# dash-robotics/perception

Hardware: AMD Instinct MI355X
Metric: frames/sec (640x480 D435 cloud, plane+cluster+ICP) (higher is better)
Workload: dtype f32

## Files before the change

perception_amd/csrc/common.hpp:

```cpp
#pragma once
#include <hip/hip_runtime.h>
#include <stdint.h>

#include "../../include/cuboid_hip.h"

namespace cd {

constexpr int WAVE = 64;
constexpr int BLOCK = 256;
constexpr int WAVES_PER_BLOCK = BLOCK / WAVE;
constexpr int ITEMS = 8;
constexpr int TILE = BLOCK * ITEMS;
constexpr int WAVE_SPAN = WAVE * ITEMS;
constexpr int RADIX_BITS = 8;
constexpr int RADIX = 1 << RADIX_BITS;
#ifndef CD_SORT_BLOCK
#define CD_SORT_BLOCK 1024
#endif
constexpr int SORT_BLOCK = CD_SORT_BLOCK;
constexpr int SORT_TILE = SORT_BLOCK * ITEMS;
#ifndef CD_SCATTER_BLOCK
#define CD_SCATTER_BLOCK 512
#endif
constexpr int SCATTER_BLOCK = CD_SCATTER_BLOCK;
constexpr int SCATTER_TILE = SCATTER_BLOCK * ITEMS;
constexpr int RUN_SHIFT = 20;
constexpr uint32_t RUN_START_MASK = (1u << RUN_SHIFT) - 1u;
constexpr int KICP = CD_MAX_CLUSTERS_PER_FRAME;
constexpr int FIX_SHIFT = 32;
constexpr int FIX_SHIFT_D2 = 36;
constexpr int RND_TABLE = 1 << 15;
constexpr int SAMPLER_MAP = 8192;
constexpr int MAX_HYP = 1024 + 16;
constexpr int CELL_BUCKETS = 1 << 16;
constexpr int ICP_TPL_CHUNK = 2048;
constexpr int ICP_SUB = 64;
#ifndef CD_PIPE_SLOTS
#define CD_PIPE_SLOTS 4
#endif
static_assert(CD_PIPE_SLOTS >= 1 && CD_PIPE_SLOTS <= 6, "LDS budget of k_icp_pipe");
constexpr int ICP_TPL_LDS = CD_PIPE_SLOTS <= 2 ? 7616 : 7552;
constexpr int ICP_MAX_CELLS = 12288;
constexpr int ICP_CELL_STRIDE = ICP_MAX_CELLS + 8;
constexpr int ICP_MAX_CHUNKS = 12;
constexpr int ICP_BIG_MAX = 65535;
constexpr int ICP_BIG_PATCHES = 1024;
constexpr int ICP_QSLICE = 512;

struct FrameState {
    int32_t status;
    int32_t n_c;
    uint32_t mn[3], mx[3];
    int32_t min_b[3], div_b[3];
    int32_t key_bits;
    int32_t n_v;
    int32_t n_plane;
    int32_t n_o;
    int32_t n_k;
    int32_t n_hyp;
    int32_t sampler_exhausted;
    int32_t ksize[KICP];
    int32_t koff[KICP];
    float origin[3];
    int32_t n_cropped;
    int32_t cl_done;
    int32_t crop_overflow;
    int32_t scan_stalled;
    int32_t n_runs;
    int32_t digit_vary;
    int32_t pad_;
};

struct CropLimits {
    float zlo, zhi, xlo, xhi;
};

struct KeyPack {
    int32_t enabled;
    int32_t bi, bj;
    int32_t ilo, jlo, klo;
};

struct BBoxGate {
    double P[12];
    float rect[4];
    int32_t enable;
    int32_t pad;
};

struct IcpCluster {
    int32_t src_off;
    int32_t n;
    int32_t frame, k;
    int32_t tpl_off, tpl_m;
    int32_t tile0;
    int32_t slot;
};

struct IcpGrid {
    float ox, oy, oz, inv;
    float cell;
    int32_t nx, ny, nz;
    int32_t ncell;
    int32_t cell_off;
    int32_t kd_split;
    int32_t pad;
    float half_lo[2][4], half_hi[2][4];
    int32_t nchunk;
    int32_t chunk_start[ICP_MAX_CHUNKS], chunk_n[ICP_MAX_CHUNKS];
    int32_t pad2[3];
    float chunk_lo[ICP_MAX_CHUNKS][4], chunk_hi[ICP_MAX_CHUNKS][4];
};

struct IcpSuper {
    int32_t n;
    int32_t first[64], cnt[64];
    float lo[64][4], hi[64][4];
};

constexpr int LAT_MAX_FACES = 6;
constexpr int LAT_MAX_TAB = 512;
struct IcpLattice {
    int32_t nface;
    int32_t ntab;
    int32_t n[3];
    int32_t toff[3];
    float noi[3], inv[3];
    int32_t w[LAT_MAX_FACES];
    int32_t fast[LAT_MAX_FACES];
    int32_t base[LAT_MAX_FACES];
    float c[LAT_MAX_FACES];
    uint32_t m0[LAT_MAX_FACES], m1[LAT_MAX_FACES], m2[LAT_MAX_FACES];
    int32_t axis_face[3];
    float axis_c[3];
    int32_t axes_distinct;
    float4 tab[LAT_MAX_TAB];
};

inline void lattice_classify_axes(IcpLattice* L) {
    uint32_t nan_bits = 0x7fc00000u;
    float nan;
    static_assert(sizeof(nan) == sizeof(nan_bits), "float32");
    __builtin_memcpy(&nan, &nan_bits, sizeof(nan));
    for (int a = 0; a < 3; ++a) { L->axis_face[a] = -1; L->axis_c[a] = nan; }
    L->axes_distinct = 0;
    if (L->nface < 1 || L->nface > 3) return;
    for (int f = 0; f < L->nface; ++f) {
        const int w = L->w[f];
        if (w < 0 || w > 2 || L->axis_face[w] >= 0) {
            for (int a = 0; a < 3; ++a) { L->axis_face[a] = -1; L->axis_c[a] = nan; }
            return;
        }
        L->axis_face[w] = f; L->axis_c[w] = L->c[f];
    }
    L->axes_distinct = 1;
}

struct IcpState {
    float Tfinal[16];
    float T[16];
    double prev_mse;
    int32_t iters;
    int32_t done;
    int32_t converged;
    int32_t status;
};

struct IcpWork {
    int32_t cluster, tile;
};

struct IcpParams {
    int32_t max_iter;
    float grid_rc;
    double trans_eps, rel_mse, rot_thr, abs_mse;
    int32_t pipe_slots;
    int32_t donate;
    int32_t* don;
    int32_t don_idle;
    int32_t don_fault;
};
struct IcpBound {
    float d2_max;
    int32_t bounded;
    uint32_t* ncorr;
};
constexpr int DON_AVAIL = 0;
constexpr int DON_FINISHED = 1;
constexpr int DON_TAIL = 2;
constexpr int DON_HEAD = 3;
constexpr int DON_ERR = 4;
constexpr int DON_BOX = 16;
constexpr int DON_CAP = 2048;

#ifdef __HIPCC__
#ifndef CD_NO_FRONT_PRIO
#define CD_FRONT_PRIO() __builtin_amdgcn_s_setprio(3)
#else
#define CD_FRONT_PRIO()
#endif
__device__ __forceinline__ uint32_t f2ord(float f) {
    const uint32_t u = __float_as_uint(f);
    return (u & 0x80000000u) ? ~u : (u | 0x80000000u);
}
__host__ __device__ __forceinline__ float ord2f(uint32_t o) {
    const uint32_t u = (o & 0x80000000u) ? (o & 0x7fffffffu) : ~o;
#ifdef __HIP_DEVICE_COMPILE__
    return __uint_as_float(u);
#else
    float f;
    __builtin_memcpy(&f, &u, 4);
    return f;
#endif
}
__device__ __forceinline__ uint64_t ballot64(bool p) { return __builtin_amdgcn_ballot_w64(p); }
#ifdef CD_BOUNDS
__device__ __forceinline__ bool cd_in_range(bool ok, unsigned code) {
    if (!ok) printf("cuboid_hip BOUNDS: check %u failed in workgroup %u thread %u\n", code, (unsigned)blockIdx.x, (unsigned)threadIdx.x);
    return ok;
}
#define CD_IN_RANGE(cond, code) cd::cd_in_range((cond), (code))
#else
#define CD_IN_RANGE(cond, code) true
#endif
template <int R, typename T>
__device__ __forceinline__ void load_rows_clamped(const T* __restrict__ a, int first, int n, T (&v)[R]) {
#pragma unroll
    for (int j = 0; j < R; ++j) {
        int e = first + j * WAVE;
        e = e < n ? e : n - 1;
        v[j] = a[e < 0 ? 0 : e];
    }
}

__device__ __forceinline__ uint64_t lanemask_lt() {
    const uint32_t lane = threadIdx.x & 63;
    return (lane == 0) ? 0ull : (~0ull >> (64 - lane));
}
template <int R>
__device__ __forceinline__ int tile_prefix(const uint64_t (&bal)[R], int (&s_cnt)[WAVES_PER_BLOCK], int* total) {
    const int w = threadIdx.x >> 6, lane = threadIdx.x & 63;
    int wtot = 0;
#pragma unroll
    for (int j = 0; j < R; ++j) wtot += __popcll(bal[j]);
    __syncthreads();
    if (lane == 0) s_cnt[w] = wtot;
    __syncthreads();
    int pos = 0, tot = 0;
    for (int q = 0; q < WAVES_PER_BLOCK; ++q) { if (q < w) pos += s_cnt[q]; tot += s_cnt[q]; }
    *total = tot;
    return pos;
}
__device__ __forceinline__ long long fixq(float v, int shift) {
    return __double2ll_rn(ldexp((double)v, shift));
}
__device__ __forceinline__ unsigned long long fixq_fast(float v, int shift) {
    const double u = __dadd_rn(ldexp((double)v, shift), 6755399441055744.0);
    const unsigned long long b = (unsigned long long)__double_as_longlong(u);
    const int hi = __builtin_amdgcn_sbfe((int)(unsigned)(b >> 32), 0, 19);
    return ((unsigned long long)(unsigned)hi << 32) | (unsigned)b;
}
#define CD_DPP_ADD2(a, b, ctrl)                                                                                   \
    asm volatile("s_nop 1\n\t"                                                                                    \
                 "v_add_co_u32_dpp %0, vcc, %0, %0 " ctrl " row_mask:0xf bank_mask:0xf bound_ctrl:0\n\t"         \
                 "v_addc_co_u32_dpp %1, vcc, %1, %1, vcc " ctrl " row_mask:0xf bank_mask:0xf bound_ctrl:0\n\t"   \
                 "v_add_co_u32_dpp %2, vcc, %2, %2 " ctrl " row_mask:0xf bank_mask:0xf bound_ctrl:0\n\t"         \
                 "v_addc_co_u32_dpp %3, vcc, %3, %3, vcc " ctrl " row_mask:0xf bank_mask:0xf bound_ctrl:0"        \
                 : "+v"(a##lo), "+v"(a##hi), "+v"(b##lo), "+v"(b##hi)::"vcc")
__device__ __forceinline__ void wave_fold_to_lds(const unsigned long long (&S)[16], int nsum, unsigned long long* dst) {
    const int lane = threadIdx.x & 63;
#pragma unroll
    for (int k = 0; k < 16; k += 2) {
        if (k < nsum) {
            unsigned xlo = (unsigned)S[k], xhi = (unsigned)(S[k] >> 32), ylo = (unsigned)S[k + 1], yhi = (unsigned)(S[k + 1] >> 32);
            CD_DPP_ADD2(x, y, "row_shr:1");
            CD_DPP_ADD2(x, y, "row_shr:2");
            CD_DPP_ADD2(x, y, "row_shr:4");
            CD_DPP_ADD2(x, y, "row_shr:8");
            if ((lane & 15) == 15) {
                atomicAdd(&dst[k], ((unsigned long long)xhi << 32) | xlo);
                if (k + 1 < nsum) atomicAdd(&dst[k + 1], ((unsigned long long)yhi << 32) | ylo);
            }
        }
    }
}

__device__ __forceinline__ unsigned long long wave_sum_u64(unsigned long long v) {
#pragma unroll
    for (int o = 32; o > 0; o >>= 1) v += __shfl_xor(v, o, 64);
    return v;
}
__device__ __forceinline__ int wave_sum_i32(int v) {
#pragma unroll
    for (int o = 32; o > 0; o >>= 1) v += __shfl_xor(v, o, 64);
    return v;
}
__device__ __forceinline__ float dist2(float ax, float ay, float az, float bx, float by, float bz) {
    const float dx = ax - bx, dy = ay - by, dz = az - bz;
    return __fadd_rn(__fadd_rn(__fmul_rn(dx, dx), __fmul_rn(dy, dy)), __fmul_rn(dz, dz));
}
constexpr int TICKET_PITCH = 32;
__device__ __forceinline__ int take_ticket(int* counter, int tickets, int* s_ticket) {
    if (threadIdx.x == 0) {
        const int t = __hip_atomic_fetch_add(counter, 1, __ATOMIC_RELAXED, __HIP_MEMORY_SCOPE_AGENT);
        if (t == tickets - 1) __hip_atomic_store(counter, 0, __ATOMIC_RELAXED, __HIP_MEMORY_SCOPE_AGENT);
        *s_ticket = CD_IN_RANGE(t >= 0 && t < tickets, 1u) ? t : 0;
    }
    __syncthreads();
    return *s_ticket;
}
__device__ __forceinline__ int chained_scan(int* state, int stride, int tile, int tot, int* gave_up) {
    unsigned* st = reinterpret_cast<unsigned*>(state);
    const unsigned FLAG_TOTAL = 1u << 30, FLAG_PREFIX = 2u << 30, VALUE = (1u << 30) - 1u;
    int excl = 0;
    if (tile > 0) {
        __hip_atomic_store(st + (size_t)tile * stride, FLAG_TOTAL | (unsigned)tot, __ATOMIC_RELAXED, __HIP_MEMORY_SCOPE_AGENT);
        for (int q = tile - 1; q >= 0; --q) {
            unsigned v;
            int spins = 0;
            do {
                v = __hip_atomic_load(st + (size_t)q * stride, __ATOMIC_RELAXED, __HIP_MEMORY_SCOPE_AGENT);
                if (++spins > (1 << 20)) { *gave_up = 1; v = FLAG_PREFIX; }
            } while ((v & (FLAG_TOTAL | FLAG_PREFIX)) == 0u);
            excl += (int)(v & VALUE);
            if (v & FLAG_PREFIX) break;
        }
    }
    __hip_atomic_store(st + (size_t)tile * stride, FLAG_PREFIX | (unsigned)(excl + tot), __ATOMIC_RELAXED, __HIP_MEMORY_SCOPE_AGENT);
    return excl;
}
__device__ __forceinline__ void chained_scan2(unsigned long long* state, int tile, int tot_a, int tot_b, int* excl_a, int* excl_b,
                                              int* gave_up) {
    const unsigned long long FLAG_TOTAL = 1ull << 62, FLAG_PREFIX = 2ull << 62, MASK = (1ull << 31) - 1ull;
    unsigned long long ea = 0ull, eb = 0ull;
    if (tile > 0) {
        __hip_atomic_store(state + tile, FLAG_TOTAL | ((unsigned long long)(unsigned)tot_b << 31) | (unsigned long long)(unsigned)tot_a,
                           __ATOMIC_RELAXED, __HIP_MEMORY_SCOPE_AGENT);
        for (int q = tile - 1; q >= 0; --q) {
            unsigned long long v;
            int spins = 0;
            do {
                v = __hip_atomic_load(state + q, __ATOMIC_RELAXED, __HIP_MEMORY_SCOPE_AGENT);
                if (++spins > (1 << 20)) { *gave_up = 1; v = FLAG_PREFIX; }
            } while ((v & (FLAG_TOTAL | FLAG_PREFIX)) == 0ull);
            ea += v & MASK;
            eb += (v >> 31) & MASK;
            if (v & FLAG_PREFIX) break;
        }
    }
    __hip_atomic_store(state + tile, FLAG_PREFIX | ((eb + (unsigned long long)(unsigned)tot_b) << 31) | (ea + (unsigned long long)(unsigned)tot_a),
                       __ATOMIC_RELAXED, __HIP_MEMORY_SCOPE_AGENT);
    *excl_a = (int)ea;
    *excl_b = (int)eb;
}
__device__ __forceinline__ float plane_dist(float a, float b, float c, float d, float x, float y, float z) {
    return fabsf(__fadd_rn(__fadd_rn(__fmul_rn(a, x), __fmul_rn(b, y)), __fadd_rn(__fmul_rn(c, z), d)));
}
#endif

}
```

perception_amd/csrc/k_plane.hip:

```cpp
#include <algorithm>

#include "extract_flags.hpp"
#include "kernels.hpp"

namespace cd {

constexpr int SAMPLER_MAP_SMALL = 1024;
constexpr int SAMPLER_SMALL_HYP = 64;
static_assert(3 * (SAMPLER_SMALL_HYP - 1) + 3 + 6 <= (SAMPLER_MAP_SMALL * 3) / 4,
              "the small map holds the slots of SAMPLER_SMALL_HYP hypotheses without a rejected sample: 3 + 3 (h - 1) before the last draw, which asks for 6 more");
static_assert(2 * SAMPLER_MAP_SMALL * sizeof(int) <= 8 * 1024 && 2 * SAMPLER_MAP <= CELL_BUCKETS, "8 KiB of LDS; the spill area is the frame's part of the cluster hash heads");

struct SamplerState {
    int rp, h, used, it, exhausted;
};

template <int MAP>
__device__ __forceinline__ bool sampler_run(int* key, int* val, SamplerState& st, const float4* __restrict__ P, int n,
                                            const int* __restrict__ rnd, int h_target, float4* __restrict__ M, int* __restrict__ V) {
    auto slot = [&](int pos) {
        uint32_t h = ((uint32_t)pos * 2654435761u) & (MAP - 1);
        while (key[h] != -1 && key[h] != pos) h = (h + 1) & (MAP - 1);
        return (int)h;
    };
    int rp = st.rp, h = st.h, used = st.used, it0 = st.it, exhausted = 0;
    auto get = [&](int pos) { const int h = slot(pos); return key[h] == pos ? val[h] : pos; };
    auto set = [&](int pos, int v) { const int h = slot(pos); if (key[h] == -1) ++used; key[h] = pos; val[h] = v; };
    while (h < h_target) {
        bool good = false;
        int s0 = 0, s1 = 0, s2 = 0;
        for (int it = it0; it < 1000; ++it) {
            if (rp + 3 > RND_TABLE || used + 6 > (SAMPLER_MAP * 3) / 4) { exhausted = 1; break; }
            if (MAP < SAMPLER_MAP && used + 6 > (MAP * 3) / 4) { st.rp = rp; st.h = h; st.used = used; st.it = it; return false; }
            for (int i = 0; i < 3; ++i) {
                const uint32_t r = (uint32_t)rnd[rp++];
                const int j = i + (int)(r % (uint32_t)(n - i));
                const int vi = get(i), vj = get(j);
                set(i, vj); set(j, vi);
            }
            s0 = get(0); s1 = get(1); s2 = get(2);
            const float4 p0 = P[s0], p1 = P[s1], p2 = P[s2];
            const float q0 = __fdiv_rn(p1.x - p0.x, p2.x - p0.x);
            const float q1 = __fdiv_rn(p1.y - p0.y, p2.y - p0.y);
            const float q2 = __fdiv_rn(p1.z - p0.z, p2.z - p0.z);
            if ((q0 != q1) || (q2 != q1)) { good = true; break; }
        }
        it0 = 0;
        if (!good) { exhausted = 1; break; }
        const float4 p0 = P[s0], p1 = P[s1], p2 = P[s2];
        const float ax = p1.x - p0.x, ay = p1.y - p0.y, az = p1.z - p0.z;
        const float bx = p2.x - p0.x, by = p2.y - p0.y, bz = p2.z - p0.z;
        const float q0 = __fdiv_rn(ax, bx), q1 = __fdiv_rn(ay, by), q2 = __fdiv_rn(az, bz);
        int ok = 1;
        float4 m = make_float4(0.f, 0.f, 0.f, 0.f);
        if (q0 == q1 && q2 == q1) {
            ok = 0;
        } else {
            float mx = __fsub_rn(__fmul_rn(ay, bz), __fmul_rn(az, by));
            float my = __fsub_rn(__fmul_rn(az, bx), __fmul_rn(ax, bz));
            float mz = __fsub_rn(__fmul_rn(ax, by), __fmul_rn(ay, bx));
            const float nrm = __fsqrt_rn(__fadd_rn(__fadd_rn(__fmul_rn(mx, mx), __fmul_rn(my, my)), __fmul_rn(mz, mz)));
            mx = __fdiv_rn(mx, nrm); my = __fdiv_rn(my, nrm); mz = __fdiv_rn(mz, nrm);
            const float d = __fmul_rn(-1.0f, __fadd_rn(__fadd_rn(__fmul_rn(mx, p0.x), __fmul_rn(my, p0.y)), __fmul_rn(mz, p0.z)));
            m = make_float4(mx, my, mz, d);
        }
        M[h] = m;
        V[h] = ok;
        ++h;
    }
    st.rp = rp; st.h = h; st.used = used; st.it = 0; st.exhausted = exhausted;
    return true;
}

template <int MAP>
__global__ void __launch_bounds__(WAVE) k_ransac_sample(const float4* __restrict__ vox, int N,
                                                        FrameState* __restrict__ fs, const int* __restrict__ rnd,
                                                        int h_target, const int* __restrict__ active,
                                                        float4* __restrict__ models, int* __restrict__ valid,
                                                        int* __restrict__ spill, int spill_pitch) {
    CD_FRONT_PRIO();
    __shared__ int s_key[MAP];
    __shared__ int s_val[MAP];
    const int f = blockIdx.x;
    if (active && !active[f]) return;
    for (int i = threadIdx.x; i < MAP; i += WAVE) s_key[i] = -1;
    __syncthreads();
    if (threadIdx.x != 0) return;
    const int n = fs[f].n_v;
    const float4* P = vox + (size_t)f * N;
    float4* M = models + (size_t)f * MAX_HYP;
    int* V = valid + (size_t)f * MAX_HYP;
    if (n < 3) { fs[f].n_hyp = 0; fs[f].sampler_exhausted = 1; return; }
    SamplerState st = {0, 0, 0, 0, 0};
    const bool finished = sampler_run<MAP>(s_key, s_val, st, P, n, rnd, h_target, M, V);
    if (MAP < SAMPLER_MAP && !finished) {
        int* g_key = spill + (size_t)f * spill_pitch;
        int* g_val = g_key + SAMPLER_MAP;
        for (int i = 0; i < SAMPLER_MAP; ++i) g_key[i] = -1;
        for (int i = 0; i < MAP; ++i) {
            const int pos = s_key[i];
            if (pos == -1) continue;
            uint32_t h = ((uint32_t)pos * 2654435761u) & (SAMPLER_MAP - 1);
            while (g_key[h] != -1) h = (h + 1) & (SAMPLER_MAP - 1);
            g_key[h] = pos;
            g_val[h] = s_val[i];
        }
        sampler_run<SAMPLER_MAP>(g_key, g_val, st, P, n, rnd, h_target, M, V);
    }
    fs[f].n_hyp = st.h;
    fs[f].sampler_exhausted = st.exhausted;
}

__global__ void __launch_bounds__(BLOCK) k_ransac_count(const float4* __restrict__ vox, int N,
                                                        const FrameState* __restrict__ fs,
                                                        const float4* __restrict__ models, const int* __restrict__ valid,
                                                        const int* __restrict__ active, int h0, int h1, float thr,
                                                        int* __restrict__ counts) {
    CD_FRONT_PRIO();
    const int f = blockIdx.y, tile = blockIdx.x, w = threadIdx.x >> 6, lane = threadIdx.x & 63;
    if (active && !active[f]) return;
    const int n = fs[f].n_v;
    if (tile * TILE >= n) return;
    const int hmax = min(h1, fs[f].n_hyp);
    const float4* P = vox + (size_t)f * N;
    const int base = tile * TILE + w * WAVE_SPAN + lane;
    float px[ITEMS], py[ITEMS], pz[ITEMS];
    bool in[ITEMS];
#pragma unroll
    for (int j = 0; j < ITEMS; ++j) {
        const int e = base + j * WAVE;
        in[j] = e < n;
        const float4 p = P[e < n ? e : n - 1];
        px[j] = p.x; py[j] = p.y; pz[j] = p.z;
    }
    const float4* M = models + (size_t)f * MAX_HYP;
    const int* V = valid + (size_t)f * MAX_HYP;
    for (int h = h0; h < hmax; ++h) {
        if (!V[h]) continue;
        const float4 m = M[h];
        int c = 0;
#pragma unroll
        for (int j = 0; j < ITEMS; ++j)
            c += __popcll(__ballot(in[j] && plane_dist(m.x, m.y, m.z, m.w, px[j], py[j], pz[j]) < thr));
        if (lane == 0 && c) atomicAdd(&counts[(size_t)f * MAX_HYP + h], c);
    }
}

__global__ void __launch_bounds__(BLOCK) k_plane_cov(const float4* __restrict__ vox, int N,
                                                     const FrameState* __restrict__ fs, const float4* __restrict__ model,
                                                     const int* __restrict__ have, float thr,
                                                     unsigned long long* __restrict__ sums) {
    CD_FRONT_PRIO();
    const int f = blockIdx.y, tile = blockIdx.x, w = threadIdx.x >> 6, lane = threadIdx.x & 63;
    const int n = fs[f].n_v;
    if (tile * TILE >= n || !have[f]) return;
    const float4 m = model[f];
    const float4* P = vox + (size_t)f * N;
    const int base = tile * TILE + w * WAVE_SPAN + lane;
    unsigned long long S[10] = {0, 0, 0, 0, 0, 0, 0, 0, 0, 0};
    float4 pr[ITEMS];
    load_rows_clamped<ITEMS>(P, base, n, pr);
#pragma unroll
    for (int j = 0; j < ITEMS; ++j) {
        const int e = base + j * WAVE;
        if (e < n) {
            const float4 p = pr[j];
            if (plane_inlier(m, 1, thr, p)) {
                S[0] += (unsigned long long)fixq(__fmul_rn(p.x, p.x), FIX_SHIFT);
                S[1] += (unsigned long long)fixq(__fmul_rn(p.x, p.y), FIX_SHIFT);
                S[2] += (unsigned long long)fixq(__fmul_rn(p.x, p.z), FIX_SHIFT);
                S[3] += (unsigned long long)fixq(__fmul_rn(p.y, p.y), FIX_SHIFT);
                S[4] += (unsigned long long)fixq(__fmul_rn(p.y, p.z), FIX_SHIFT);
                S[5] += (unsigned long long)fixq(__fmul_rn(p.z, p.z), FIX_SHIFT);
                S[6] += (unsigned long long)fixq(p.x, FIX_SHIFT);
                S[7] += (unsigned long long)fixq(p.y, FIX_SHIFT);
                S[8] += (unsigned long long)fixq(p.z, FIX_SHIFT);
                S[9] += 1ull;
            }
        }
    }
#pragma unroll
    for (int k = 0; k < 10; ++k) {
        const unsigned long long t = wave_sum_u64(S[k]);
        if (lane == 0 && t) atomicAdd(&sums[(size_t)f * 10 + k], t);
    }
}

__global__ void __launch_bounds__(BLOCK) k_plane_flag_count(const float4* __restrict__ vox, int N, int T,
                                                            const FrameState* __restrict__ fs,
                                                            const float4* __restrict__ model, const int* __restrict__ have,
                                                            float thr, int negative, int crop2, float z2lo, float z2hi, BBoxGate gate,
                                                            FrameRects rects, int* __restrict__ cnt_plane, int* __restrict__ cnt_obj) {
    CD_FRONT_PRIO();
    __shared__ int s_a[WAVES_PER_BLOCK], s_b[WAVES_PER_BLOCK];
    const int f = blockIdx.y, tile = blockIdx.x, w = threadIdx.x >> 6, lane = threadIdx.x & 63;
    const int n = fs[f].n_v;
    if (tile * TILE >= n) return;
    frame_rect(gate, rects, f);
    const float4 m = model[f];
    const int hv = have[f];
    const float4* P = vox + (size_t)f * N;
    const int base = tile * TILE + w * WAVE_SPAN + lane;
    int ca = 0, cb = 0;
    float4 pr[ITEMS];
    load_rows_clamped<ITEMS>(P, base, n, pr);
#pragma unroll
    for (int j = 0; j < ITEMS; ++j) {
        const int e = base + j * WAVE;
        bool inl = false, obj = false;
        if (e < n) extract_flags(m, hv, thr, negative, crop2, z2lo, z2hi, gate, pr[j], inl, obj);
        ca += __popcll(__ballot(inl));
        cb += __popcll(__ballot(obj));
    }
    if (lane == 0) { s_a[w] = ca; s_b[w] = cb; }
    __syncthreads();
    if (threadIdx.x == 0) {
        cnt_plane[(size_t)f * T + tile] = s_a[0] + s_a[1] + s_a[2] + s_a[3];
        cnt_obj[(size_t)f * T + tile] = s_b[0] + s_b[1] + s_b[2] + s_b[3];
    }
}

__global__ void __launch_bounds__(BLOCK) k_extract_scatter(const float4* __restrict__ vox, int N, int T,
                                                           const FrameState* __restrict__ fs,
                                                           const float4* __restrict__ model, const int* __restrict__ have,
                                                           float thr, int negative, int crop2, float z2lo, float z2hi, BBoxGate gate,
                                                           FrameRects rects, const int* __restrict__ off_plane, const int* __restrict__ off_obj,
                                                           int* __restrict__ plane_idx, float4* __restrict__ obj_out) {
    CD_FRONT_PRIO();
    __shared__ int s_a[WAVES_PER_BLOCK], s_b[WAVES_PER_BLOCK];
    const int f = blockIdx.y, tile = blockIdx.x, w = threadIdx.x >> 6, lane = threadIdx.x & 63;
    const int n = fs[f].n_v;
    if (tile * TILE >= n) return;
    frame_rect(gate, rects, f);
    const size_t fbase = (size_t)f * N;
    const float4 m = model[f];
    const int hv = have[f];
    const float4* P = vox + fbase;
    const int base = tile * TILE + w * WAVE_SPAN + lane;
    float4 p[ITEMS];
    uint64_t ba[ITEMS], bb[ITEMS];
    int ca = 0, cb = 0;
    load_rows_clamped<ITEMS>(P, base, n, p);
#pragma unroll
    for (int j = 0; j < ITEMS; ++j) {
        const int e = base + j * WAVE;
        bool inl = false, obj = false;
        if (e < n) extract_flags(m, hv, thr, negative, crop2, z2lo, z2hi, gate, p[j], inl, obj);
        ba[j] = __ballot(inl);
        bb[j] = __ballot(obj);
        ca += __popcll(ba[j]);
        cb += __popcll(bb[j]);
    }
    if (lane == 0) { s_a[w] = ca; s_b[w] = cb; }
    __syncthreads();
    int pa = off_plane[(size_t)f * T + tile], pb = off_obj[(size_t)f * T + tile];
    for (int q = 0; q < w; ++q) { pa += s_a[q]; pb += s_b[q]; }
    const uint64_t lt = lanemask_lt();
#pragma unroll
    for (int j = 0; j < ITEMS; ++j) {
        const int e = base + j * WAVE;
        if ((ba[j] >> lane) & 1ull) plane_idx[fbase + pa + __popcll(ba[j] & lt)] = e;
        if ((bb[j] >> lane) & 1ull) obj_out[fbase + pb + __popcll(bb[j] & lt)] = p[j];
        pa += __popcll(ba[j]);
        pb += __popcll(bb[j]);
    }
}

void launch_ransac_sample(hipStream_t s, const float4* vox, int N, int F, FrameState* fs, const int* rnd_table,
                          int h_target, const int* active, float4* models, int* valid, int* spill, int spill_pitch) {
    if (spill && spill_pitch >= 2 * SAMPLER_MAP && h_target <= SAMPLER_SMALL_HYP)
        hipLaunchKernelGGL(k_ransac_sample<SAMPLER_MAP_SMALL>, dim3(F), dim3(WAVE), 0, s, vox, N, fs, rnd_table, h_target, active, models, valid, spill, spill_pitch);
    else
        hipLaunchKernelGGL(k_ransac_sample<SAMPLER_MAP>, dim3(F), dim3(WAVE), 0, s, vox, N, fs, rnd_table, h_target, active, models, valid, spill, spill_pitch);
}
void launch_ransac_count(hipStream_t s, const float4* vox, int N, int F, int Tact, const FrameState* fs,
                         const float4* models, const int* valid, const int* active, int h0, int h1, float thr, int* counts) {
    hipLaunchKernelGGL(k_ransac_count, dim3(Tact, F), dim3(BLOCK), 0, s, vox, N, fs, models, valid, active, h0, h1, thr, counts);
}
void launch_plane_cov(hipStream_t s, const float4* vox, int N, int F, int Tact, const FrameState* fs, const float4* model,
                      const int* have, float thr, unsigned long long* sums) {
    hipLaunchKernelGGL(k_plane_cov, dim3(Tact, F), dim3(BLOCK), 0, s, vox, N, fs, model, have, thr, sums);
}
void launch_plane_flag_count(hipStream_t s, const float4* vox, int N, int F, int T, int Tact, const FrameState* fs,
                             const float4* model, const int* have, float thr, int negative, int crop2, float z2lo,
                             float z2hi, const BBoxGate& gate, const FrameRects& rects, int* cnt_plane, int* cnt_obj) {
    hipLaunchKernelGGL(k_plane_flag_count, dim3(Tact, F), dim3(BLOCK), 0, s, vox, N, T, fs, model, have, thr, negative,
                       crop2, z2lo, z2hi, gate, rects, cnt_plane, cnt_obj);
}
void launch_extract_scatter(hipStream_t s, const float4* vox, int N, int F, int T, int Tact, const FrameState* fs,
                            const float4* model, const int* have, float thr, int negative, int crop2, float z2lo,
                            float z2hi, const BBoxGate& gate, const FrameRects& rects, const int* off_plane, const int* off_obj, int* plane_idx,
                            float4* obj) {
    hipLaunchKernelGGL(k_extract_scatter, dim3(Tact, F), dim3(BLOCK), 0, s, vox, N, T, fs, model, have, thr, negative,
                       crop2, z2lo, z2hi, gate, rects, off_plane, off_obj, plane_idx, obj);
}

__global__ void __launch_bounds__(BLOCK) k_mark_indices(const int* __restrict__ idx, int m, int n, int* __restrict__ flag) {
    CD_FRONT_PRIO();
    const int i = blockIdx.x * BLOCK + threadIdx.x;
    if (i < m) { const int k = idx[i]; if (k >= 0 && k < n) flag[k] = 1; }
}
__global__ void __launch_bounds__(BLOCK) k_passthrough_mark(const char* __restrict__ in, size_t stride, int n, int field_off, double lo, double hi,
                                                            int negative, int* __restrict__ flag) {
    CD_FRONT_PRIO();
    const int i = blockIdx.x * BLOCK + threadIdx.x;
    if (i >= n) return;
    const char* p = in + (size_t)i * stride;
    const float x = *reinterpret_cast<const float*>(p), y = *reinterpret_cast<const float*>(p + 4), z = *reinterpret_cast<const float*>(p + 8);
    bool remove = !((fabsf(x) <= 3.402823466e38f) && (fabsf(y) <= 3.402823466e38f) && (fabsf(z) <= 3.402823466e38f));
    if (field_off >= 0) {
        const float vf = *reinterpret_cast<const float*>(p + field_off);
        const double v = (double)vf;
        remove = remove || !(fabsf(vf) <= 3.402823466e38f);
        remove = remove || (negative ? (v < hi && v > lo) : (v > hi || v < lo));
    }
    flag[i] = remove ? 1 : 0;
}
__global__ void __launch_bounds__(BLOCK) k_select_unmarked(const int* __restrict__ flag, int n, int* __restrict__ state,
                                                           FrameState* __restrict__ fs, int* __restrict__ out, int* __restrict__ ticket) {
    CD_FRONT_PRIO();
    __shared__ int s_cnt[WAVES_PER_BLOCK];
    __shared__ int s_excl, s_ticket;
    const int tile = take_ticket(ticket, (int)gridDim.x, &s_ticket), w = threadIdx.x >> 6, lane = threadIdx.x & 63;
    const int base = tile * TILE + w * WAVE_SPAN;
    uint64_t bal[ITEMS];
    int wtot = 0;
    int fl[ITEMS];
    load_rows_clamped<ITEMS>(flag, base + lane, n, fl);
#pragma unroll
    for (int j = 0; j < ITEMS; ++j) {
        const int e = base + j * WAVE + lane;
        bal[j] = ballot64(e < n && fl[j] == 0);
        wtot += __popcll(bal[j]);
    }
    if (lane == 0) s_cnt[w] = wtot;
    __syncthreads();
    if (threadIdx.x == 0) {
        int tot = 0;
        for (int k = 0; k < WAVES_PER_BLOCK; ++k) tot += s_cnt[k];
        const int excl = chained_scan(state, 1, tile, tot, &fs[0].scan_stalled);
        s_excl = excl;
        if ((tile + 1) * TILE >= n) fs[0].n_plane = excl + tot;
    }
    __syncthreads();
    int pos = s_excl;
    for (int k = 0; k < w; ++k) pos += s_cnt[k];
    const uint64_t lt = lanemask_lt();
#pragma unroll
    for (int j = 0; j < ITEMS; ++j) {
        if ((bal[j] >> lane) & 1ull) out[pos + __popcll(bal[j] & lt)] = base + j * WAVE + lane;
        pos += __popcll(bal[j]);
    }
}
__global__ void __launch_bounds__(BLOCK) k_gather_records(const uint32_t* __restrict__ in, int words, const int* __restrict__ idx,
                                                          int m, uint32_t* __restrict__ out) {
    CD_FRONT_PRIO();
    const size_t t = (size_t)blockIdx.x * BLOCK + threadIdx.x;
    if (t >= (size_t)m * words) return;
    const int r = (int)(t / words), wd = (int)(t % words);
    out[t] = in[(size_t)idx[r] * words + wd];
}
__global__ void __launch_bounds__(BLOCK) k_pack_records(const float4* __restrict__ pts, int m, int words, int rgb_word, uint32_t pad3,
                                                        uint32_t* __restrict__ out) {
    CD_FRONT_PRIO();
    const size_t t = (size_t)blockIdx.x * BLOCK + threadIdx.x;
    if (t >= (size_t)m * words) return;
    const int r = (int)(t / words), wd = (int)(t % words);
    const float4 p = pts[r];
    uint32_t v = 0u;
    if (wd == 0) v = __float_as_uint(p.x);
    else if (wd == 1) v = __float_as_uint(p.y);
    else if (wd == 2) v = __float_as_uint(p.z);
    else if (wd == rgb_word) v = __float_as_uint(p.w);
    else if (wd == 3) v = pad3;
    out[t] = v;
}
void launch_pack_records(hipStream_t s, const float4* pts, int m, int words, int rgb_word, uint32_t pad3, void* out) {
    const size_t tot = (size_t)m * words;
    if (tot > 0) hipLaunchKernelGGL(k_pack_records, dim3((unsigned)((tot + BLOCK - 1) / BLOCK)), dim3(BLOCK), 0, s, pts, m, words, rgb_word, pad3, (uint32_t*)out);
}
__global__ void __launch_bounds__(BLOCK) k_copy_rows(CopyList L) {
    CD_FRONT_PRIO();
    const CopySeg sg = L.seg[blockIdx.y];
    for (int r = blockIdx.z; r < sg.rows; r += gridDim.z)
        for (int i = blockIdx.x * BLOCK + threadIdx.x; i < sg.width_w; i += gridDim.x * BLOCK) sg.dst[(size_t)r * sg.dpitch_w + i] = sg.src[(size_t)r * sg.spitch_w + i];
}
__global__ void __launch_bounds__(BLOCK) k_zero_regions(ZeroRegions r) {
    CD_FRONT_PRIO();
    if ((int)blockIdx.y == r.n) {
        constexpr size_t W = sizeof(FrameState) / 4, MN0 = offsetof(FrameState, mn) / 4;
        uint32_t* p = reinterpret_cast<uint32_t*>(r.fs);
        const size_t n = W * (size_t)r.nfs;
        for (size_t i = (size_t)blockIdx.x * BLOCK + threadIdx.x; i < n; i += (size_t)gridDim.x * BLOCK) {
            const size_t w = i % W;
            p[i] = (w >= MN0 && w < MN0 + 3) ? 0xffffffffu : 0u;
        }
        return;
    }
    uint32_t* p = r.ptr[blockIdx.y];
    const size_t n = r.words[blockIdx.y];
    for (size_t i = (size_t)blockIdx.x * BLOCK + threadIdx.x; i < n; i += (size_t)gridDim.x * BLOCK) p[i] = 0u;
}
void launch_zero_regions(hipStream_t s, const ZeroRegions& r) {
    const int ny = r.n + (r.fs && r.nfs > 0 ? 1 : 0);
    if (ny > 0) hipLaunchKernelGGL(k_zero_regions, dim3(128, ny), dim3(BLOCK), 0, s, r);
}
void launch_copy_list(hipStream_t s, const CopyList& L) {
    if (L.n <= 0) return;
    int gx = 1, gz = 1;
    for (int k = 0; k < L.n; ++k) {
        gx = std::max(gx, std::min(64, (L.seg[k].width_w + BLOCK - 1) / BLOCK));
        gz = std::max(gz, std::min(L.seg[k].rows, 256));
    }
    hipLaunchKernelGGL(k_copy_rows, dim3(gx, L.n, gz), dim3(BLOCK), 0, s, L);
}
void launch_copy_rows(hipStream_t s, void* dst, size_t dpitch, const void* src, size_t spitch, size_t width, int rows) {
    if (width == 0 || rows <= 0) return;
    CopyList L;
    L.n = 1;
    L.seg[0] = CopySeg{(uint32_t*)dst, (const uint32_t*)src, dpitch / 4, spitch / 4, (int)(width / 4), rows};
    launch_copy_list(s, L);
}
void launch_passthrough_mark(hipStream_t s, const void* in, size_t stride, int n, int field_off, double lo, double hi, int negative, int* flag) {
    if (n > 0) hipLaunchKernelGGL(k_passthrough_mark, dim3((n + BLOCK - 1) / BLOCK), dim3(BLOCK), 0, s, (const char*)in, stride, n, field_off, lo, hi, negative, flag);
}
void launch_mark_indices(hipStream_t s, const int* idx, int m, int n, int* flag) {
    if (m > 0) hipLaunchKernelGGL(k_mark_indices, dim3((m + BLOCK - 1) / BLOCK), dim3(BLOCK), 0, s, idx, m, n, flag);
}
void launch_select_unmarked(hipStream_t s, const int* flag, int n, int* state, FrameState* fs, int* out, int* ticket) {
    hipLaunchKernelGGL(k_select_unmarked, dim3((n + TILE - 1) / TILE), dim3(BLOCK), 0, s, flag, n, state, fs, out, ticket);
}
void launch_gather_records(hipStream_t s, const void* in, int words, const int* idx, int m, void* out) {
    const size_t tot = (size_t)m * words;
    if (tot > 0) hipLaunchKernelGGL(k_gather_records, dim3((unsigned)((tot + BLOCK - 1) / BLOCK)), dim3(BLOCK), 0, s, (const uint32_t*)in, words, idx, m, (uint32_t*)out);
}

}
```

perception_amd/csrc/k_sort.hip:

```cpp
#include "kernels.hpp"

namespace cd {

constexpr int SORT_WAVES = SORT_BLOCK / WAVE;
constexpr int SCATTER_WAVES = SCATTER_BLOCK / WAVE;
static_assert(SCATTER_BLOCK % WAVE == 0 && SCATTER_BLOCK <= 1024, "whole waves, one workgroup");
static_assert(RADIX <= SCATTER_BLOCK && RADIX % WAVE == 0, "one thread per bin for the prefix over waves and bins; s_ws / s_gs hold one word per wave of bins");
static_assert(WAVE_SPAN <= 0xffff && SCATTER_TILE <= 0xffff, "a wave's bin counts and their prefix over the tile's waves are kept as unsigned short");

struct KeyGrid {
    float mb0, mb1, mb2;
    int d0, d01;
};
__device__ __forceinline__ KeyGrid key_grid(const FrameState& s) {
    KeyGrid g;
    g.mb0 = (float)s.min_b[0]; g.mb1 = (float)s.min_b[1]; g.mb2 = (float)s.min_b[2];
    g.d0 = s.div_b[0]; g.d01 = s.div_b[0] * s.div_b[1];
    return g;
}
__device__ __forceinline__ uint32_t voxel_key(uint32_t a, const KeyPack& kp, const KeyGrid& g) {
    const int fx = (int)(a & ((1u << kp.bi) - 1u)) + kp.ilo;
    const int fy = (int)((a >> kp.bi) & ((1u << kp.bj) - 1u)) + kp.jlo;
    const int fz = (int)(a >> (kp.bi + kp.bj)) + kp.klo;
    const int i0 = (int)__fsub_rn((float)fx, g.mb0), i1 = (int)__fsub_rn((float)fy, g.mb1), i2 = (int)__fsub_rn((float)fz, g.mb2);
    return (uint32_t)(i0 + i1 * g.d0 + i2 * g.d01);
}

#ifdef CD_SORTDBG
__device__ unsigned long long g_sort_dbg[8];
extern "C" int cd_debug_sort(unsigned long long* out, int reset) {
    if (hipMemcpyFromSymbol(out, HIP_SYMBOL(g_sort_dbg), sizeof(g_sort_dbg)) != hipSuccess) return -1;
    if (reset) { static unsigned long long z[8]; (void)hipMemcpyToSymbol(HIP_SYMBOL(g_sort_dbg), z, sizeof(z)); }
    return 0;
}
#define SORT_PHASE(k) { __syncthreads(); if (threadIdx.x == 0) { const unsigned long long t_ = wall_clock64(); atomicAdd(&g_sort_dbg[k], t_ - t0_); t0_ = t_; } }
#else
#define SORT_PHASE(k)
#endif
constexpr int SORT_MAX_PASSES = 4;
constexpr int GHIST_TILES = 4;

__global__ void __launch_bounds__(SORT_BLOCK) k_radix_ghist(const uint32_t* __restrict__ kin, int N, int npass,
                                                            const FrameState* __restrict__ fs, uint32_t* __restrict__ ghist,
                                                            KeyPack kp) {
    CD_FRONT_PRIO();
    __shared__ uint32_t s_h[SORT_MAX_PASSES][RADIX];
    const int f = blockIdx.y, lane = threadIdx.x & 63;
    const int n = fs[f].n_c;
    const int e0 = blockIdx.x * GHIST_TILES * SORT_TILE;
    if (e0 >= n) return;
    for (int q = threadIdx.x; q < SORT_MAX_PASSES * RADIX; q += SORT_BLOCK) (&s_h[0][0])[q] = 0;
    __syncthreads();
    const uint32_t* k = kin + (size_t)f * N;
    const KeyGrid g = key_grid(fs[f]);
    for (int t = 0; t < GHIST_TILES; ++t) {
        const int base = e0 + t * SORT_TILE + (threadIdx.x >> 6) * WAVE_SPAN + lane;
        if (e0 + t * SORT_TILE >= n) break;
#pragma unroll
        for (int j = 0; j < ITEMS; ++j) {
            const int e = base + j * WAVE;
            const bool valid = e < n;
            uint32_t key = 0;
            if (valid) key = kp.enabled ? voxel_key(k[e], kp, g) : k[e];
            for (int p = 0; p < npass; ++p) {
                const uint32_t d = valid ? ((key >> (p * RADIX_BITS)) & (RADIX - 1)) : 0xffffffffu;
                const uint32_t prev = (uint32_t)__shfl_up((int)d, 1, 64);
                const uint64_t heads = __ballot(lane == 0 || d != prev);
                const uint64_t above = lane == 63 ? 0ull : heads & ~((2ull << lane) - 1ull);
                const int next = above ? __ffsll((long long)above) - 1 : 64;
                if (((heads >> lane) & 1ull) && valid) atomicAdd(&s_h[p][d], (uint32_t)(next - lane));
            }
        }
    }
    __syncthreads();
    for (int q = threadIdx.x; q < npass * RADIX; q += SORT_BLOCK) {
        const uint32_t c = (&s_h[0][0])[q];
        if (c) atomicAdd(&ghist[(size_t)f * SORT_MAX_PASSES * RADIX + q], c);
    }
}

__global__ void __launch_bounds__(SCATTER_BLOCK) k_radix_scatter(const uint32_t* __restrict__ kin, const uint32_t* __restrict__ vin,
                                                         uint32_t* __restrict__ kout, uint32_t* __restrict__ vout, int N,
                                                         int T, int Tact, int pass, int shift, FrameState* __restrict__ fs,
                                                         const uint32_t* __restrict__ ghist, int* __restrict__ state,
                                                         KeyPack kp, int use_runs, int* __restrict__ ticket) {
    CD_FRONT_PRIO();
    __shared__ int s_ticket;
    __shared__ unsigned short s_wh[SCATTER_WAVES][RADIX];
    __shared__ uint32_t s_goff[RADIX];
    __shared__ uint32_t s_bstart[RADIX];
    __shared__ uint32_t s_k[SCATTER_TILE], s_v[SCATTER_TILE];
    __shared__ uint32_t s_ws[RADIX / WAVE], s_gs[RADIX / WAVE];
    const int F = gridDim.x / Tact;
    const int f = blockIdx.x % F, tile = take_ticket(ticket + f * TICKET_PITCH, Tact, &s_ticket), w = threadIdx.x >> 6, lane = threadIdx.x & 63;
    const int n = use_runs ? fs[f].n_runs : fs[f].n_c;
    if (tile * SCATTER_TILE >= n) return;
    const size_t fbase = (size_t)f * N;
#ifdef CD_SORTDBG
    unsigned long long t0_ = wall_clock64();
    if (threadIdx.x == 0) atomicAdd(&g_sort_dbg[7], 1ull);
#endif
    for (int q = threadIdx.x; q < SCATTER_WAVES * RADIX; q += SCATTER_BLOCK) (&s_wh[0][0])[q] = 0;
    __syncthreads();
    const int base = tile * SCATTER_TILE + w * WAVE_SPAN + lane;
    const uint64_t lt = lanemask_lt();
    const KeyGrid g = key_grid(fs[f]);
    uint32_t key[ITEMS], rank[ITEMS], val[ITEMS];
#pragma unroll
    for (int j = 0; j < ITEMS; ++j) {
        const int e = base + j * WAVE;
        key[j] = e < n ? kin[fbase + e] : 0xffffffffu;
        val[j] = e < n ? (vin ? vin[fbase + e] : (uint32_t)e) : 0u;
    }
#pragma unroll
    for (int j = 0; j < ITEMS; ++j) {
        const int e = base + j * WAVE;
        const bool valid = e < n;
        if (kp.enabled && valid) key[j] = voxel_key(key[j], kp, g);
        const uint32_t d = (key[j] >> shift) & (RADIX - 1);
        uint32_t dl = 0u, dh = 0u;
#pragma unroll
        for (int b = 0; b < RADIX_BITS; ++b) {
            const int y = (int)(d << (31 - b)) >> 31;
            const uint64_t m = __ballot(y < 0);
            dl |= (uint32_t)m ^ (uint32_t)y;
            dh |= (uint32_t)(m >> 32) ^ (uint32_t)y;
        }
        const uint64_t peers = ~(((uint64_t)dh << 32) | dl) & __ballot(valid);
        uint32_t bin_base = 0;
        if (valid) bin_base = s_wh[w][d];
        if (valid && (peers >> lane) == 1ull) s_wh[w][d] = (unsigned short)(bin_base + (uint32_t)__popcll(peers));
        rank[j] = bin_base + (uint32_t)__popcll(peers & lt);
    }
    __syncthreads();
    SORT_PHASE(0)
    if (threadIdx.x < RADIX) {
        const int d = threadIdx.x;
        uint32_t run = 0;
#pragma unroll
        for (int q = 0; q < SCATTER_WAVES; ++q) {
            const uint32_t c = s_wh[q][d];
            s_wh[q][d] = (unsigned short)run;
            run += c;
        }
        const uint32_t tot = ghist[((size_t)f * SORT_MAX_PASSES + pass) * RADIX + d];
        uint32_t inc = run, ginc = tot;
#pragma unroll
        for (int o = 1; o < 64; o <<= 1) {
            const uint32_t u = __shfl_up(inc, o, 64), gu = __shfl_up(ginc, o, 64);
            if (lane >= o) { inc += u; ginc += gu; }
        }
        if (lane == 63) { s_ws[w] = inc; s_gs[w] = ginc; }
        s_bstart[d] = inc - run;
        const int before = chained_scan(state + (size_t)f * T * RADIX + d, RADIX, tile, (int)run, &fs[f].scan_stalled);
        s_goff[d] = ginc - tot + (uint32_t)before;
    }
    __syncthreads();
    if (threadIdx.x < RADIX) {
        uint32_t add = 0, gadd = 0;
        for (int q = 0; q < w; ++q) { add += s_ws[q]; gadd += s_gs[q]; }
        s_bstart[threadIdx.x] += add;
        s_goff[threadIdx.x] += gadd;
    }
    __syncthreads();
    SORT_PHASE(1)
#pragma unroll
    for (int j = 0; j < ITEMS; ++j) {
        const int e = base + j * WAVE;
        if (e < n) {
            const uint32_t d = (key[j] >> shift) & (RADIX - 1);
            const uint32_t lp = s_bstart[d] + s_wh[w][d] + rank[j];
            if (CD_IN_RANGE(lp < (uint32_t)SCATTER_TILE, 2u)) {
                s_k[lp] = key[j];
                s_v[lp] = val[j];
            }
        }
    }
    __syncthreads();
    SORT_PHASE(2)
    const int cnt = min(SCATTER_TILE, n - tile * SCATTER_TILE);
#pragma unroll
    for (int j = 0; j < ITEMS; ++j) {
        const int lp = threadIdx.x + j * SCATTER_BLOCK;
        if (lp < cnt) {
            const uint32_t k = s_k[lp];
            const uint32_t d = (k >> shift) & (RADIX - 1);
            const uint32_t dst = s_goff[d] + ((uint32_t)lp - s_bstart[d]);
            if (CD_IN_RANGE(dst < (uint32_t)n, 3u)) {
                kout[fbase + dst] = k;
                vout[fbase + dst] = s_v[lp];
            }
        }
    }
    SORT_PHASE(3)
}

int launch_radix_sort(hipStream_t s, uint32_t* const key[2], uint32_t* const val[2], int N, int F, int Tact, int Tscat, int npass,
                      FrameState* fs, uint32_t* ghist, int* state, KeyPack kp, int* ticket) {
    if (npass <= 0) return 0;
    if (hipMemsetAsync(ghist, 0, sizeof(uint32_t) * (size_t)F * SORT_MAX_PASSES * RADIX, s) != hipSuccess) return -1;
    if (hipMemsetAsync(state, 0, sizeof(int) * (size_t)npass * F * Tscat * RADIX, s) != hipSuccess) return -1;
    const int G = (Tact + GHIST_TILES - 1) / GHIST_TILES;
    hipLaunchKernelGGL(k_radix_ghist, dim3(G, F), dim3(SORT_BLOCK), 0, s, key[0], N, npass, fs, ghist, kp);
    int cur = 0;
    for (int pass = 0; pass < npass; ++pass) {
        hipLaunchKernelGGL(k_radix_scatter, dim3(Tscat * F), dim3(SCATTER_BLOCK), 0, s, key[cur], pass ? val[cur] : nullptr, key[cur ^ 1],
                           val[cur ^ 1], N, Tscat, Tscat, pass, pass * RADIX_BITS, fs, ghist, state + (size_t)pass * F * Tscat * RADIX, kp, 0, ticket);
        kp.enabled = 0;
        cur ^= 1;
    }
    return cur;
}

__global__ void __launch_bounds__(SORT_BLOCK) k_voxel_runs(const uint32_t* __restrict__ kin, int N, int T, int Tact, int npass,
                                                           FrameState* __restrict__ fs, uint32_t* __restrict__ ghist,
                                                           int* __restrict__ state, uint32_t* __restrict__ kout,
                                                           uint32_t* __restrict__ vout, KeyPack kp, int* __restrict__ ticket) {
    CD_FRONT_PRIO();
    __shared__ uint32_t s_h[SORT_MAX_PASSES][RADIX];
    __shared__ int s_cnt[SORT_WAVES];
    __shared__ int s_out0, s_ticket;
    const int F = gridDim.x / Tact;
    const int f = blockIdx.x % F, tile = take_ticket(ticket + f * TICKET_PITCH, Tact, &s_ticket), w = threadIdx.x >> 6, lane = threadIdx.x & 63;
    const int n = fs[f].n_c;
    if (tile * SORT_TILE >= n) return;
    for (int q = threadIdx.x; q < SORT_MAX_PASSES * RADIX; q += SORT_BLOCK) (&s_h[0][0])[q] = 0;
    const size_t fbase = (size_t)f * N;
    const uint32_t* k = kin + fbase;
    const KeyGrid g = key_grid(fs[f]);
    const int base = tile * SORT_TILE + w * WAVE_SPAN + lane;
    uint32_t key[ITEMS];
    uint64_t heads[ITEMS];
    int nvalid[ITEMS], wtot = 0;
#pragma unroll
    for (int j = 0; j < ITEMS; ++j) {
        const int e = base + j * WAVE;
        const bool valid = e < n;
        key[j] = 0xffffffffu;
        if (valid) key[j] = kp.enabled ? voxel_key(k[e], kp, g) : k[e];
        const uint32_t prev = (uint32_t)__shfl_up((int)key[j], 1, 64);
        heads[j] = __ballot(valid && (lane == 0 || key[j] != prev));
        nvalid[j] = __popcll(__ballot(valid));
        wtot += __popcll(heads[j]);
    }
    if (lane == 0) s_cnt[w] = wtot;
    __syncthreads();
    int pos = 0, nheads = 0;
    for (int q = 0; q < SORT_WAVES; ++q) { if (q < w) pos += s_cnt[q]; nheads += s_cnt[q]; }
    if (threadIdx.x == 0) {
        const int excl = chained_scan(state + (size_t)f * T, 1, tile, nheads, &fs[f].scan_stalled);
        s_out0 = excl;
        if ((tile + 1) * SORT_TILE >= n) fs[f].n_runs = excl + nheads;
    }
    __syncthreads();
    const int out0 = s_out0;
    const uint64_t lt = lanemask_lt();
#pragma unroll
    for (int j = 0; j < ITEMS; ++j) {
        const bool is_head = (heads[j] >> lane) & 1ull;
        if (is_head) {
            const uint64_t above = lane == 63 ? 0ull : heads[j] & ~((2ull << lane) - 1ull);
            const int next = above ? __ffsll((long long)above) - 1 : nvalid[j];
            const size_t o = fbase + (size_t)(out0 + pos + __popcll(heads[j] & lt));
            kout[o] = key[j];
            vout[o] = (uint32_t)(base + j * WAVE) | ((uint32_t)(next - lane) << RUN_SHIFT);
        }
        if (heads[j]) {
            const int first = __ffsll((long long)heads[j]) - 1;
            for (int p = 0; p < npass; ++p) {
                const uint32_t d = (key[j] >> (p * RADIX_BITS)) & (RADIX - 1);
                if (p > 0) {
                    const uint32_t d0 = (uint32_t)__builtin_amdgcn_readlane((int)d, first);
                    if (__ballot(is_head && d != d0) == 0ull) {
                        if (lane == first) atomicAdd(&s_h[p][d0], (uint32_t)__popcll(heads[j]));
                        continue;
                    }
                }
                if (is_head) atomicAdd(&s_h[p][d], 1u);
            }
        }
        pos += __popcll(heads[j]);
    }
    __syncthreads();
    for (int q = threadIdx.x; q < npass * RADIX; q += SORT_BLOCK) {
        const uint32_t c = (&s_h[0][0])[q];
        if (c) atomicAdd(&ghist[(size_t)f * SORT_MAX_PASSES * RADIX + q], c);
    }
}

int launch_radix_sort_runs(hipStream_t s, uint32_t* const key[2], uint32_t* const val[2], int N, int F, int T, int Tact, int Tscat, int npass,
                           FrameState* fs, uint32_t* ghist, int* state, int* tile_state, KeyPack kp, int* ticket) {
    if (npass <= 0) return 0;
    if (hipMemsetAsync(ghist, 0, sizeof(uint32_t) * (size_t)F * SORT_MAX_PASSES * RADIX, s) != hipSuccess) return -1;
    if (hipMemsetAsync(state, 0, sizeof(int) * (size_t)npass * F * Tscat * RADIX, s) != hipSuccess) return -1;
    if (hipMemsetAsync(tile_state, 0, sizeof(int) * (size_t)F * T, s) != hipSuccess) return -1;
    hipLaunchKernelGGL(k_voxel_runs, dim3(Tact * F), dim3(SORT_BLOCK), 0, s, key[0], N, T, Tact, npass, fs, ghist, tile_state, key[1],
                       val[1], kp, ticket);
    kp.enabled = 0;
    int cur = 1;
    for (int pass = 0; pass < npass; ++pass) {
        hipLaunchKernelGGL(k_radix_scatter, dim3(Tscat * F), dim3(SCATTER_BLOCK), 0, s, key[cur], val[cur], key[cur ^ 1], val[cur ^ 1], N,
                           Tscat, Tscat, pass, pass * RADIX_BITS, fs, ghist, state + (size_t)pass * F * Tscat * RADIX, kp, 1, ticket);
        cur ^= 1;
    }
    return cur;
}

int launch_radix_scatter_runs(hipStream_t s, uint32_t* const key[2], uint32_t* const val[2], int N, int F, int Tact, const int* digits, int ndigits,
                              FrameState* fs, const uint32_t* ghist, int* state, int* ticket) {
    if (ndigits <= 0) return 0;
    if (hipMemsetAsync(state, 0, sizeof(int) * (size_t)ndigits * F * Tact * RADIX, s) != hipSuccess) return -1;
    KeyPack none;
    none.enabled = 0; none.bi = none.bj = 0; none.ilo = none.jlo = none.klo = 0;
    int cur = 0;
    for (int q = 0; q < ndigits; ++q) {
        hipLaunchKernelGGL(k_radix_scatter, dim3(Tact * F), dim3(SCATTER_BLOCK), 0, s, key[cur], val[cur], key[cur ^ 1], val[cur ^ 1], N,
                           Tact, Tact, digits[q], digits[q] * RADIX_BITS, fs, ghist, state + (size_t)q * F * Tact * RADIX, none, 1, ticket);
        cur ^= 1;
    }
    return cur;
}

}
```

perception_amd/csrc/k_voxel.hip:

```cpp
#include "kernels.hpp"

namespace cd {

template <int R>
__device__ __forceinline__ void load_rows(const char* __restrict__ in, size_t stride, size_t fbase, int first, int N, int rgb_off,
                                          float (&x)[R], float (&y)[R], float (&z)[R], uint32_t (&rgb)[R]) {
    if (stride == 16 && rgb_off == 12) {
        float4 v[R];
#pragma unroll
        for (int j = 0; j < R; ++j) v[j] = *reinterpret_cast<const float4*>(in + (fbase + (size_t)min(first + j * WAVE, N - 1)) * 16);
#pragma unroll
        for (int j = 0; j < R; ++j) { x[j] = v[j].x; y[j] = v[j].y; z[j] = v[j].z; rgb[j] = __float_as_uint(v[j].w); }
    } else {
#pragma unroll
        for (int j = 0; j < R; ++j) {
            const char* p = in + (fbase + (size_t)min(first + j * WAVE, N - 1)) * stride;
            x[j] = *reinterpret_cast<const float*>(p);
            y[j] = *reinterpret_cast<const float*>(p + 4);
            z[j] = *reinterpret_cast<const float*>(p + 8);
            rgb[j] = rgb_off >= 0 ? *reinterpret_cast<const uint32_t*>(p + rgb_off) : 0u;
        }
    }
}

__device__ __forceinline__ bool crop_keep(float x, float y, float z, const CropLimits& L) {
    const bool fin = (fabsf(x) <= 3.402823466e38f) && (fabsf(y) <= 3.402823466e38f) && (fabsf(z) <= 3.402823466e38f);
    return fin && z >= L.zlo && z <= L.zhi && x >= L.xlo && x <= L.xhi;
}

struct CropBox {
    float mn[3] = {3.402823466e38f, 3.402823466e38f, 3.402823466e38f};
    float mx[3] = {-3.402823466e38f, -3.402823466e38f, -3.402823466e38f};
    __device__ __forceinline__ void add(float x, float y, float z) {
        mn[0] = fminf(mn[0], x); mn[1] = fminf(mn[1], y); mn[2] = fminf(mn[2], z);
        mx[0] = fmaxf(mx[0], x); mx[1] = fmaxf(mx[1], y); mx[2] = fmaxf(mx[2], z);
    }
    __device__ __forceinline__ void reduce_wave(float (&s_mn)[3], float (&s_mx)[3], int lane) {
#pragma unroll
        for (int a = 0; a < 3; ++a) {
#pragma unroll
            for (int o = 32; o > 0; o >>= 1) {
                mn[a] = fminf(mn[a], __shfl_xor(mn[a], o, 64));
                mx[a] = fmaxf(mx[a], __shfl_xor(mx[a], o, 64));
            }
        }
        if (lane == 0) {
            for (int a = 0; a < 3; ++a) { s_mn[a] = mn[a]; s_mx[a] = mx[a]; }
        }
    }
    static __device__ __forceinline__ void commit(FrameState& s, const float (&s_mn)[WAVES_PER_BLOCK][3],
                                                  const float (&s_mx)[WAVES_PER_BLOCK][3], int tot) {
        if (tot <= 0) return;
        for (int a = 0; a < 3; ++a) {
            float lo = s_mn[0][a], hi = s_mx[0][a];
            for (int k = 1; k < WAVES_PER_BLOCK; ++k) { lo = fminf(lo, s_mn[k][a]); hi = fmaxf(hi, s_mx[k][a]); }
            atomicMin(&s.mn[a], f2ord(lo));
            atomicMax(&s.mx[a], f2ord(hi));
        }
    }
};

__device__ __forceinline__ uint32_t packed_cell_key(float x, float y, float z, float inv, const KeyPack& kp, bool* fits) {
    const float jlo = (float)kp.jlo, jhi = (float)(kp.jlo + ((1 << kp.bj) - 1));
    const float fy = floorf(__fmul_rn(y, inv));
    *fits = fy >= jlo && fy <= jhi;
    const uint32_t ui = (uint32_t)((int)floorf(__fmul_rn(x, inv)) - kp.ilo);
    const uint32_t uj = *fits ? (uint32_t)((int)fy - kp.jlo) : 0u;
    const uint32_t uk = (uint32_t)((int)floorf(__fmul_rn(z, inv)) - kp.klo);
    return ui | (uj << kp.bi) | (uk << (kp.bi + kp.bj));
}

__global__ void __launch_bounds__(BLOCK) k_crop_count(const char* __restrict__ in, size_t stride, int N, int rgb_off,
                                                      CropLimits lim, int T, FrameState* __restrict__ fs,
                                                      int* __restrict__ tile_cnt) {
    CD_FRONT_PRIO();
    __shared__ int s_cnt[WAVES_PER_BLOCK];
    __shared__ float s_mn[WAVES_PER_BLOCK][3], s_mx[WAVES_PER_BLOCK][3];
    const int f = blockIdx.y, tile = blockIdx.x, w = threadIdx.x >> 6, lane = threadIdx.x & 63;
    const size_t fbase = (size_t)f * N;
    const int base = tile * TILE + w * WAVE_SPAN;
    int cnt = 0;
    CropBox box;
    float qx[ITEMS], qy[ITEMS], qz[ITEMS];
    uint32_t qc[ITEMS];
    load_rows<ITEMS>(in, stride, fbase, base + lane, N, rgb_off, qx, qy, qz, qc);
#pragma unroll
    for (int j = 0; j < ITEMS; ++j) {
        const int e = base + j * WAVE + lane;
        bool keep = false;
        if (e < N) {
            keep = crop_keep(qx[j], qy[j], qz[j], lim);
            if (keep) box.add(qx[j], qy[j], qz[j]);
        }
        cnt += __popcll(__ballot(keep));
    }
    box.reduce_wave(s_mn[w], s_mx[w], lane);
    if (lane == 0) s_cnt[w] = cnt;
    __syncthreads();
    if (threadIdx.x == 0) {
        int tot = 0;
        for (int k = 0; k < WAVES_PER_BLOCK; ++k) tot += s_cnt[k];
        tile_cnt[(size_t)f * T + tile] = tot;
        CropBox::commit(fs[f], s_mn, s_mx, tot);
    }
}

__global__ void __launch_bounds__(BLOCK) k_scan_tiles(ScanJob j0, ScanJob j1, int T, int total_pitch) {
    CD_FRONT_PRIO();
    __shared__ int s_w[WAVES_PER_BLOCK];
    __shared__ int s_base;
    const ScanJob job = blockIdx.y ? j1 : j0;
    const int row = blockIdx.x, w = threadIdx.x >> 6, lane = threadIdx.x & 63;
    int* c = job.counts + (size_t)row * T;
    if (threadIdx.x == 0) s_base = 0;
    __syncthreads();
    for (int t0 = 0; t0 < T; t0 += BLOCK) {
        const int t = t0 + threadIdx.x;
        const int v = t < T ? c[t] : 0;
        int inc = v;
#pragma unroll
        for (int o = 1; o < 64; o <<= 1) {
            const int u = __shfl_up(inc, o, 64);
            if (lane >= o) inc += u;
        }
        if (lane == 63) s_w[w] = inc;
        __syncthreads();
        int wb = 0;
        for (int k = 0; k < w; ++k) wb += s_w[k];
        const int base = s_base;
        if (t < T) c[t] = base + wb + inc - v;
        __syncthreads();
        if (threadIdx.x == BLOCK - 1) s_base = base + wb + inc;
        __syncthreads();
    }
    if (threadIdx.x == 0) {
        if (job.totals) job.totals[(size_t)row * total_pitch] = s_base;
        if (job.mirror) job.mirror[(size_t)row * total_pitch] = s_base;
    }
}

__device__ __forceinline__ void voxel_setup_frame(FrameState& s, float leaf) {
    s.key_bits = 0;
    s.n_cropped = s.n_c;
    s.origin[0] = s.origin[1] = s.origin[2] = 0.f;
    for (int a = 0; a < 3; ++a) { s.min_b[a] = 0; s.div_b[a] = 0; }
    if (s.n_c <= 0) return;
    const float inv = __fdiv_rn(1.0f, leaf);
    float mn[3], mx[3];
    for (int a = 0; a < 3; ++a) { mn[a] = ord2f(s.mn[a]); mx[a] = ord2f(s.mx[a]); s.origin[a] = mn[a]; }
    const long long dx = (long long)__fmul_rn(__fsub_rn(mx[0], mn[0]), inv) + 1;
    const long long dy = (long long)__fmul_rn(__fsub_rn(mx[1], mn[1]), inv) + 1;
    const long long dz = (long long)__fmul_rn(__fsub_rn(mx[2], mn[2]), inv) + 1;
    long long cells = 1;
    bool bad = (dx * dy * dz) > 2147483647ll;
    for (int a = 0; a < 3; ++a) {
        const int lo = (int)floorf(__fmul_rn(mn[a], inv));
        const int hi = (int)floorf(__fmul_rn(mx[a], inv));
        s.min_b[a] = lo;
        s.div_b[a] = hi - lo + 1;
        cells *= (long long)(hi - lo + 1);
        if (cells > 2147483647ll) bad = true;
    }
    if (bad) { s.status = CD_ERR_LEAF_TOO_SMALL; s.n_c = 0; s.n_runs = 0; return; }
    int bits = 1;
    while (bits < 31 && (1ll << bits) < cells) ++bits;
    s.key_bits = bits;
}
__global__ void __launch_bounds__(WAVE) k_voxel_setup(FrameState* __restrict__ fs, float leaf, const uint32_t* __restrict__ ghist,
                                                      FrameState* __restrict__ mirror) {
    CD_FRONT_PRIO();
    const int f = blockIdx.x, lane = threadIdx.x;
    int vary = 0;
    if (ghist) {
        for (int d = 0; d < 4; ++d) {
            int bins = 0;
            for (int q = 0; q < RADIX / WAVE; ++q) bins += __popcll(__ballot(ghist[((size_t)f * 4 + d) * RADIX + q * WAVE + lane] != 0u));
            if (bins > 1) vary |= 1 << d;
        }
    }
    if (lane != 0) return;
    FrameState s = fs[f];
    if (ghist) s.digit_vary = vary;
    voxel_setup_frame(s, leaf);
    fs[f] = s;
    if (mirror) mirror[f] = s;
}

__global__ void __launch_bounds__(BLOCK) k_crop_compact(const char* __restrict__ in, size_t stride, int N, int pitch,
                                                        int rgb_off, CropLimits lim, int T, float leaf,
                                                        const FrameState* __restrict__ fs,
                                                        const int* __restrict__ tile_off, float4* __restrict__ cpt,
                                                        uint32_t* __restrict__ keys) {
    CD_FRONT_PRIO();
    __shared__ int s_cnt[WAVES_PER_BLOCK];
    const int f = blockIdx.y, tile = blockIdx.x, w = threadIdx.x >> 6, lane = threadIdx.x & 63;
    if (fs[f].n_c <= 0) return;
    const size_t fbase = (size_t)f * N;
    const size_t obase = (size_t)f * pitch;
    const int base = tile * TILE + w * WAVE_SPAN;
    float px[ITEMS], py[ITEMS], pz[ITEMS];
    uint32_t pc[ITEMS];
    uint64_t bal[ITEMS];
    int wtot = 0;
    load_rows<ITEMS>(in, stride, fbase, base + lane, N, rgb_off, px, py, pz, pc);
#pragma unroll
    for (int j = 0; j < ITEMS; ++j) {
        const int e = base + j * WAVE + lane;
        const bool keep = e < N && crop_keep(px[j], py[j], pz[j], lim);
        bal[j] = __ballot(keep);
        wtot += __popcll(bal[j]);
    }
    if (lane == 0) s_cnt[w] = wtot;
    __syncthreads();
    int pos = tile_off[(size_t)f * T + tile];
    for (int k = 0; k < w; ++k) pos += s_cnt[k];
    const float inv = __fdiv_rn(1.0f, leaf);
    const int mb0 = fs[f].min_b[0], mb1 = fs[f].min_b[1], mb2 = fs[f].min_b[2];
    const int d0 = fs[f].div_b[0], d01 = fs[f].div_b[0] * fs[f].div_b[1];
    const uint64_t lt = lanemask_lt();
#pragma unroll
    for (int j = 0; j < ITEMS; ++j) {
        if ((bal[j] >> lane) & 1ull) {
            const int r = pos + __popcll(bal[j] & lt);
            const int i0 = (int)__fsub_rn(floorf(__fmul_rn(px[j], inv)), (float)mb0);
            const int i1 = (int)__fsub_rn(floorf(__fmul_rn(py[j], inv)), (float)mb1);
            const int i2 = (int)__fsub_rn(floorf(__fmul_rn(pz[j], inv)), (float)mb2);
            cpt[obase + r] = make_float4(px[j], py[j], pz[j], __uint_as_float(pc[j]));
            keys[obase + r] = (uint32_t)(i0 + i1 * d0 + i2 * d01);
        }
        pos += __popcll(bal[j]);
    }
}

__global__ void __launch_bounds__(BLOCK) k_crop_fused(const char* __restrict__ in, size_t stride, int N, int pitch,
                                                      int rgb_off, CropLimits lim, int T, int Tin, float leaf, KeyPack kp,
                                                      FrameState* __restrict__ fs, int* __restrict__ state,
                                                      float4* __restrict__ cpt,
                                                      uint32_t* __restrict__ keys, int* __restrict__ ticket) {
    CD_FRONT_PRIO();
    __shared__ int s_cnt[WAVES_PER_BLOCK];
    __shared__ float s_mn[WAVES_PER_BLOCK][3], s_mx[WAVES_PER_BLOCK][3];
    __shared__ int s_excl, s_ticket;
    const int w = threadIdx.x >> 6, lane = threadIdx.x & 63;
    const int F = gridDim.x / Tin;
    const int f = blockIdx.x % F, tile = take_ticket(ticket + f * TICKET_PITCH, Tin, &s_ticket);
    const size_t fbase = (size_t)f * N;
    const size_t obase = (size_t)f * pitch;
    const int base = tile * TILE + w * WAVE_SPAN;
    float px[ITEMS], py[ITEMS], pz[ITEMS];
    uint32_t pc[ITEMS];
    uint64_t bal[ITEMS];
    int wtot = 0;
    CropBox box;
    load_rows<ITEMS>(in, stride, fbase, base + lane, N, rgb_off, px, py, pz, pc);
#pragma unroll
    for (int j = 0; j < ITEMS; ++j) {
        const int e = base + j * WAVE + lane;
        bool keep = false;
        if (e < N) {
            keep = crop_keep(px[j], py[j], pz[j], lim);
            if (keep) box.add(px[j], py[j], pz[j]);
        }
        bal[j] = __ballot(keep);
        wtot += __popcll(bal[j]);
    }
    box.reduce_wave(s_mn[w], s_mx[w], lane);
    if (lane == 0) s_cnt[w] = wtot;
    __syncthreads();
    if (threadIdx.x == 0) {
        int tot = 0;
        for (int k = 0; k < WAVES_PER_BLOCK; ++k) tot += s_cnt[k];
        const int excl = chained_scan(state + (size_t)f * T, 1, tile, tot, &fs[f].crop_overflow);
        s_excl = excl;
        if (tile == Tin - 1) fs[f].n_c = excl + tot;
        CropBox::commit(fs[f], s_mn, s_mx, tot);
    }
    __syncthreads();
    int pos = s_excl;
    for (int k = 0; k < w; ++k) pos += s_cnt[k];
    const float inv = __fdiv_rn(1.0f, leaf);
    const uint64_t lt = lanemask_lt();
    bool over = false;
#pragma unroll
    for (int j = 0; j < ITEMS; ++j) {
        if ((bal[j] >> lane) & 1ull) {
            const int r = pos + __popcll(bal[j] & lt);
            bool fits;
            const uint32_t key = packed_cell_key(px[j], py[j], pz[j], inv, kp, &fits);
            over = over || !fits;
            if (r < pitch) {
                cpt[obase + r] = make_float4(px[j], py[j], pz[j], __uint_as_float(pc[j]));
                keys[obase + r] = key;
            }
        }
        pos += __popcll(bal[j]);
    }
    if (__ballot(over) != 0ull && lane == 0) fs[f].crop_overflow = 1;
}


template <bool DIRECT>
__global__ void __launch_bounds__(BLOCK) k_crop_runs(const char* __restrict__ in, size_t stride, int N, int pitch,
                                                     int rgb_off, CropLimits lim, int T, int Tin, float leaf, KeyPack kp,
                                                     FrameState* __restrict__ fs, unsigned long long* __restrict__ state,
                                                     float4* __restrict__ cpt, uint32_t* __restrict__ rkeys, uint32_t* __restrict__ rvals,
                                                     uint32_t* __restrict__ ghist, int* __restrict__ ticket) {
    CD_FRONT_PRIO();
    __shared__ int s_cnt[WAVES_PER_BLOCK], s_rcnt[WAVES_PER_BLOCK];
    __shared__ float s_mn[WAVES_PER_BLOCK][3], s_mx[WAVES_PER_BLOCK][3];
    __shared__ uint32_t s_h[4][RADIX];
    __shared__ unsigned short s_rk[TILE];
    __shared__ uint32_t s_key[TILE];
    __shared__ int s_excl, s_rexcl, s_ticket;
    const int w = threadIdx.x >> 6, lane = threadIdx.x & 63;
    const int F = gridDim.x / Tin;
    const int f = blockIdx.x % F, tile = take_ticket(ticket + f * TICKET_PITCH, Tin, &s_ticket);
    for (int q = threadIdx.x; q < 4 * RADIX; q += BLOCK) (&s_h[0][0])[q] = 0;
    const size_t fbase = (size_t)f * N;
    const size_t obase = (size_t)f * pitch;
    const int base = tile * TILE + w * WAVE_SPAN;
    const float inv = __fdiv_rn(1.0f, leaf);
    float px[ITEMS], py[ITEMS], pz[ITEMS];
    uint32_t pc[ITEMS];
    uint64_t bal[ITEMS], heads[ITEMS];
    int wtot = 0, rtot = 0;
    CropBox box;
    bool over = false;
    load_rows<ITEMS>(in, stride, fbase, base + lane, N, rgb_off, px, py, pz, pc);
#pragma unroll
    for (int j = 0; j < ITEMS; ++j) {
        const int e = base + j * WAVE + lane;
        bool keep = false;
        uint32_t key = 0xffffffffu;
        if (e < N) {
            keep = crop_keep(px[j], py[j], pz[j], lim);
            if (keep) {
                box.add(px[j], py[j], pz[j]);
                bool fits;
                key = packed_cell_key(px[j], py[j], pz[j], inv, kp, &fits);
                over = over || !fits;
            }
        }
        bal[j] = __ballot(keep);
        const uint32_t prev = (uint32_t)__shfl_up((int)key, 1, 64);
        const bool prev_kept = lane > 0 && ((bal[j] >> (lane - 1)) & 1ull);
        heads[j] = __ballot(keep && !(prev_kept && prev == key));
        s_key[w * WAVE_SPAN + j * WAVE + lane] = key;
        wtot += __popcll(bal[j]);
        rtot += __popcll(heads[j]);
    }
    box.reduce_wave(s_mn[w], s_mx[w], lane);
    if (lane == 0) { s_cnt[w] = wtot; s_rcnt[w] = rtot; }
    __syncthreads();
    if (threadIdx.x == 0) {
        int tot = 0, rt = 0;
        for (int k = 0; k < WAVES_PER_BLOCK; ++k) { tot += s_cnt[k]; rt += s_rcnt[k]; }
        int excl = 0, rexcl = 0;
        chained_scan2(state + (size_t)f * T, tile, tot, rt, &excl, &rexcl, &fs[f].crop_overflow);
        s_excl = excl; s_rexcl = rexcl;
        if (tile == Tin - 1) { fs[f].n_c = excl + tot; fs[f].n_runs = rexcl + rt; }
        CropBox::commit(fs[f], s_mn, s_mx, tot);
    }
    __syncthreads();
    const int rexcl0 = s_rexcl;
    int pos = s_excl, rpos = rexcl0;
    for (int k = 0; k < w; ++k) { pos += s_cnt[k]; rpos += s_rcnt[k]; }
    const uint64_t lt = lanemask_lt();
#pragma unroll
    for (int j = 0; j < ITEMS; ++j) {
        const bool kept = (bal[j] >> lane) & 1ull;
        const int r = pos + __popcll(bal[j] & lt);
        if (!DIRECT && kept && r < pitch) cpt[obase + r] = make_float4(px[j], py[j], pz[j], __uint_as_float(pc[j]));
        const bool is_head = (heads[j] >> lane) & 1ull;
        if (is_head) {
            const uint64_t stop = (~bal[j] | heads[j]) & (lane == 63 ? 0ull : ~((2ull << lane) - 1ull));
            const int next = stop ? __ffsll((long long)stop) - 1 : 64;
            const int ro = rpos + __popcll(heads[j] & lt);
            const uint32_t key = s_key[w * WAVE_SPAN + j * WAVE + lane];
            s_rk[ro - rexcl0] = (unsigned short)(w * WAVE_SPAN + j * WAVE + lane);
            if (ro < pitch && CD_IN_RANGE(ro >= 0, 5u)) {
                rkeys[obase + ro] = key;
                rvals[obase + ro] = (uint32_t)(DIRECT ? base + j * WAVE + lane : r) | ((uint32_t)(next - lane) << RUN_SHIFT);
            }
        }
        pos += __popcll(bal[j]);
        rpos += __popcll(heads[j]);
    }
    if (__ballot(over) != 0ull && lane == 0) fs[f].crop_overflow = 1;
    __syncthreads();
    {
        int nr = 0;
        for (int k = 0; k < WAVES_PER_BLOCK; ++k) nr += s_rcnt[k];
        for (int q0 = w * WAVE; q0 < nr; q0 += BLOCK) {
            const int q = q0 + lane;
            const bool on = q < nr;
            const uint32_t kq = on ? s_key[s_rk[q]] : 0u;
            if (on) atomicAdd(&s_h[0][kq & (RADIX - 1)], 1u);
#pragma unroll
            for (int d = 1; d < 4; ++d) {
                const uint32_t dg = on ? ((kq >> (d * RADIX_BITS)) & (RADIX - 1)) : 0xffffffffu;
                const uint32_t prev = (uint32_t)__shfl_up((int)dg, 1, 64);
                const uint64_t hd = __ballot(lane == 0 || dg != prev);
                const uint64_t above = lane == 63 ? 0ull : hd & ~((2ull << lane) - 1ull);
                const int next = above ? __ffsll((long long)above) - 1 : 64;
                if (((hd >> lane) & 1ull) && on) atomicAdd(&s_h[d][dg], (uint32_t)(next - lane));
            }
        }
    }
    __syncthreads();
    for (int q = threadIdx.x; q < 4 * RADIX; q += BLOCK) {
        const uint32_t c = (&s_h[0][0])[q];
        if (c) atomicAdd(&ghist[(size_t)f * 4 * RADIX + q], c);
    }
}

template <int R>
__device__ __forceinline__ void head_ballots(const uint32_t* __restrict__ k, int first, int n, uint64_t (&heads)[R]) {
    const int lane = threadIdx.x & 63;
    uint32_t cur[R], left[R];
#pragma unroll
    for (int j = 0; j < R; ++j) {
        const int e = first + j * WAVE + lane;
        cur[j] = k[max(min(e, n - 1), 0)];
        left[j] = k[max(min(e - 1, n - 1), 0)];
    }
#pragma unroll
    for (int j = 0; j < R; ++j) {
        const int e = first + j * WAVE + lane;
        heads[j] = __ballot(e < n && (e == 0 || cur[j] != left[j]));
    }
}

template <int I>
__device__ __forceinline__ float quad_bcast(float v) {
    return __int_as_float(__builtin_amdgcn_update_dpp(0, __float_as_int(v), I | (I << 2) | (I << 4) | (I << 6), 0xf, 0xf, true));
}
template <int I>
__device__ __forceinline__ int quad_bcast_i(int v) {
    return __builtin_amdgcn_update_dpp(0, v, I | (I << 2) | (I << 4) | (I << 6), 0xf, 0xf, true);
}

struct TileHeads { int nheads, out0; };
__device__ __forceinline__ TileHeads tile_voxel_heads(const uint32_t* k, int n, int tile, int* state, FrameState& s,
                                                      int (&s_cnt)[WAVES_PER_BLOCK], int (&s_head)[TILE], int& s_out0) {
    const int w = threadIdx.x >> 6, lane = threadIdx.x & 63;
    const int base = tile * TILE + w * WAVE_SPAN;
    uint64_t bal[ITEMS];
    int wtot = 0;
    head_ballots<ITEMS>(k, base, n, bal);
#pragma unroll
    for (int j = 0; j < ITEMS; ++j) wtot += __popcll(bal[j]);
    if (lane == 0) s_cnt[w] = wtot;
    __syncthreads();
    int pos = 0, nheads = 0;
    for (int q = 0; q < WAVES_PER_BLOCK; ++q) { if (q < w) pos += s_cnt[q]; nheads += s_cnt[q]; }
    if (threadIdx.x == 0) {
        const int excl = chained_scan(state, 1, tile, nheads, &s.scan_stalled);
        s_out0 = excl;
        if ((tile + 1) * TILE >= n) s.n_v = excl + nheads;
    }
    const uint64_t lt = lanemask_lt();
#pragma unroll
    for (int j = 0; j < ITEMS; ++j) {
        if ((bal[j] >> lane) & 1ull) s_head[pos + __popcll(bal[j] & lt)] = base + j * WAVE + lane;
        pos += __popcll(bal[j]);
    }
    __syncthreads();
    return {nheads, s_out0};
}

__device__ __forceinline__ void rgb_add(uint32_t u, uint32_t& ir, uint32_t& ig, uint32_t& ib) {
    ir = __builtin_amdgcn_udot4(u, 0x00010000u, ir, false);
    ig = __builtin_amdgcn_udot4(u, 0x00000100u, ig, false);
    ib = __builtin_amdgcn_udot4(u, 0x00000001u, ib, false);
}
__device__ __forceinline__ void rgb_replay(const uint32_t* k, const uint32_t* v, const float4* pts,
                                           int e0, int n, uint32_t key, float& cr, float& cg, float& cb) {
    cr = cg = cb = 0.f;
    for (int e = e0; e < n && k[e] == key; ++e) {
        const uint32_t r = v[e];
        const int st = (int)(r & RUN_START_MASK), ln = (int)(r >> RUN_SHIFT);
        for (int i = 0; i < ln; ++i) {
            const uint32_t u = __float_as_uint(pts[st + i].w);
            cr += (float)((u >> 16) & 0xff); cg += (float)((u >> 8) & 0xff); cb += (float)(u & 0xff);
        }
    }
}
__device__ __forceinline__ void store_centroid(float4* vox_slot, float sx, float sy, float sz, float cr, float cg, float cb,
                                               int cnt, int rgb_on) {
    const float c = (float)cnt;
    uint32_t packed = 0;
    if (rgb_on) {
        const int R = (int)__fdiv_rn(cr, c), G = (int)__fdiv_rn(cg, c), B = (int)__fdiv_rn(cb, c);
        packed = ((uint32_t)R << 16) | ((uint32_t)G << 8) | (uint32_t)B;
    }
    *vox_slot = make_float4(__fdiv_rn(sx, c), __fdiv_rn(sy, c), __fdiv_rn(sz, c), __uint_as_float(packed));
}

__global__ void __launch_bounds__(BLOCK) k_voxel_centroid(const uint32_t* __restrict__ keys,
                                                          const uint32_t* __restrict__ vals,
                                                          const float4* __restrict__ cpt, int N, int T, int Tact, int rgb_on,
                                                          FrameState* __restrict__ fs, int* __restrict__ state,
                                                          float4* __restrict__ vox, int* __restrict__ ticket) {
    CD_FRONT_PRIO();
    __shared__ int s_cnt[WAVES_PER_BLOCK];
    __shared__ int s_head[TILE];
    __shared__ int s_out0, s_ticket;
    const int F = gridDim.x / Tact;
    const int f = blockIdx.x % F, tile = take_ticket(ticket + f * TICKET_PITCH, Tact, &s_ticket);
    const int n = fs[f].n_c;
    if (tile * TILE >= n) return;
    const size_t fbase = (size_t)f * N;
    const uint32_t* k = keys + fbase;
    const uint32_t* v = vals + fbase;
    const TileHeads th = tile_voxel_heads(k, n, tile, state + (size_t)f * T, fs[f], s_cnt, s_head, s_out0);
    const int nheads = th.nheads, out0 = th.out0;
    const int quad = threadIdx.x >> 2, ql = threadIdx.x & 3;
    for (int h = quad; h < nheads; h += BLOCK / 4) {
        const int e0 = s_head[h];
        const uint32_t key = k[e0];
        float sx = 0.f, sy = 0.f, sz = 0.f, cr = 0.f, cg = 0.f, cb = 0.f;
        int cnt = 0;
        for (int e = e0;; e += 4) {
            const int me = e + ql;
            uint32_t kk = ~key, vv = 0;
            if (me < n) { kk = k[me]; vv = v[me]; }
            const bool mine = kk == key;
            float4 p = make_float4(0.f, 0.f, 0.f, 0.f);
            if (mine) p = cpt[fbase + vv];
            const int m0 = quad_bcast_i<0>(mine), m1 = quad_bcast_i<1>(mine), m2 = quad_bcast_i<2>(mine), m3 = quad_bcast_i<3>(mine);
#define CD_ACC(I, M)                                                                                   \
            if (M) {                                                                                   \
                sx = __fadd_rn(sx, quad_bcast<I>(p.x)); sy = __fadd_rn(sy, quad_bcast<I>(p.y));        \
                sz = __fadd_rn(sz, quad_bcast<I>(p.z));                                                \
                if (rgb_on) {                                                                          \
                    const uint32_t u = __float_as_uint(quad_bcast<I>(p.w));                            \
                    cr += (float)((u >> 16) & 0xff); cg += (float)((u >> 8) & 0xff); cb += (float)(u & 0xff); \
                }                                                                                      \
                ++cnt;                                                                                 \
            }
            CD_ACC(0, m0) CD_ACC(1, m1) CD_ACC(2, m2) CD_ACC(3, m3)
#undef CD_ACC
            if (!m3) break;
        }
        if (ql == 0) store_centroid(&vox[fbase + out0 + h], sx, sy, sz, cr, cg, cb, cnt, rgb_on);
    }
}

__global__ void __launch_bounds__(BLOCK) k_voxel_centroid_runs(const uint32_t* __restrict__ keys,
                                                               const uint32_t* __restrict__ vals,
                                                               const float4* __restrict__ cpt, int N, int T, int Tact, int rgb_on,
                                                               FrameState* __restrict__ fs, int* __restrict__ state,
                                                               float4* __restrict__ vox, int* __restrict__ ticket, int pts_pitch) {
    CD_FRONT_PRIO();
    __shared__ int s_cnt[WAVES_PER_BLOCK];
    __shared__ int s_head[TILE];
    __shared__ int s_out0, s_ticket;
    const int F = gridDim.x / Tact;
    const int f = blockIdx.x % F, tile = take_ticket(ticket + f * TICKET_PITCH, Tact, &s_ticket);
    const int n = fs[f].n_runs;
    if (tile * TILE >= n) return;
    const size_t fbase = (size_t)f * N;
    const uint32_t* k = keys + fbase;
    const uint32_t* v = vals + fbase;
    const float4* pts = cpt + (size_t)f * pts_pitch;
    const TileHeads th = tile_voxel_heads(k, n, tile, state + (size_t)f * T, fs[f], s_cnt, s_head, s_out0);
    const int nheads = th.nheads, out0 = th.out0;
    const int quad = threadIdx.x >> 2, ql = threadIdx.x & 3;
    int h = quad, e0 = 0;
    uint32_t kk = 0, rec = 0;
    bool have = false;
    if (h < nheads) {
        e0 = s_head[h];
        have = e0 + ql < n;
        if (have) { kk = k[e0 + ql]; rec = v[e0 + ql]; }
    }
    while (h < nheads) {
        const int hn = h + BLOCK / 4;
        int ne0 = 0;
        uint32_t nkk = 0, nrec = 0;
        bool nhave = false;
        if (hn < nheads) {
            ne0 = s_head[hn];
            nhave = ne0 + ql < n;
            if (nhave) { nkk = k[ne0 + ql]; nrec = v[ne0 + ql]; }
        }
        const uint32_t key = (uint32_t)quad_bcast_i<0>((int)kk);
        float sx = 0.f, sy = 0.f, sz = 0.f;
        uint32_t ir = 0, ig = 0, ib = 0;
        int cnt = 0;
#define CD_ADD(P, J)                                                                                   \
        {                                                                                              \
            sx = __fadd_rn(sx, quad_bcast<J>(P.x)); sy = __fadd_rn(sy, quad_bcast<J>(P.y));            \
            sz = __fadd_rn(sz, quad_bcast<J>(P.z));                                                    \
            if (rgb_on) rgb_add(__float_as_uint(quad_bcast<J>(P.w)), ir, ig, ib);                      \
        }
#define CD_RUN(I, P, Q)                                                                                \
        if (len##I > 0) {                                                                              \
            CD_ADD(P, 0)                                                                               \
            if (len##I > 1) CD_ADD(P, 1)                                                               \
            if (len##I > 2) CD_ADD(P, 2)                                                               \
            if (len##I > 3) CD_ADD(P, 3)                                                               \
            if (len##I > 4) {                                                                          \
                CD_ADD(Q, 0)                                                                           \
                if (len##I > 5) CD_ADD(Q, 1)                                                           \
                if (len##I > 6) CD_ADD(Q, 2)                                                           \
                if (len##I > 7) CD_ADD(Q, 3)                                                           \
                for (int i = 8; i < len##I; i += 4) {    \
                    float4 t = make_float4(0.f, 0.f, 0.f, 0.f);                                        \
                    if (i + ql < len##I) t = pts[start##I + i + ql];                           \
                    CD_ADD(t, 0)                                                                       \
                    if (len##I - i > 1) CD_ADD(t, 1)                                                   \
                    if (len##I - i > 2) CD_ADD(t, 2)                                                   \
                    if (len##I - i > 3) CD_ADD(t, 3)                                                   \
                }                                                                                      \
            }                                                                                          \
        }
        for (int eb = e0;; eb += 4) {
            const int mylen = (have && kk == key) ? (int)(rec >> RUN_SHIFT) : 0, mystart = (int)(rec & RUN_START_MASK);
            const int len0 = quad_bcast_i<0>(mylen), len1 = quad_bcast_i<1>(mylen), len2 = quad_bcast_i<2>(mylen), len3 = quad_bcast_i<3>(mylen);
            const int start0 = quad_bcast_i<0>(mystart), start1 = quad_bcast_i<1>(mystart), start2 = quad_bcast_i<2>(mystart), start3 = quad_bcast_i<3>(mystart);
            uint32_t kk2 = 0, rec2 = 0;
            const bool have2 = len3 > 0 && eb + 4 + ql < n;
            if (have2) { kk2 = k[eb + 4 + ql]; rec2 = v[eb + 4 + ql]; }
            cnt += (len0 + len1) + (len2 + len3);
            float4 p0 = make_float4(0.f, 0.f, 0.f, 0.f), p1 = p0, p2 = p0, p3 = p0, q0 = p0, q1 = p0, q2 = p0, q3 = p0;
            if (ql < len0) p0 = pts[start0 + ql];
            if (ql < len1) p1 = pts[start1 + ql];
            if (ql < len2) p2 = pts[start2 + ql];
            if (ql < len3) p3 = pts[start3 + ql];
            if (4 + ql < len0) q0 = pts[start0 + 4 + ql];
            if (4 + ql < len1) q1 = pts[start1 + 4 + ql];
            if (4 + ql < len2) q2 = pts[start2 + 4 + ql];
            if (4 + ql < len3) q3 = pts[start3 + 4 + ql];
            CD_RUN(0, p0, q0) CD_RUN(1, p1, q1) CD_RUN(2, p2, q2) CD_RUN(3, p3, q3)
            if (len3 == 0) break;
            kk = kk2; rec = rec2; have = have2;
        }
#undef CD_RUN
#undef CD_ADD
        float cr = (float)ir, cg = (float)ig, cb = (float)ib;
        if (rgb_on && cnt > 65536) rgb_replay(k, v, pts, e0, n, key, cr, cg, cb);
        if (ql == 0) {
            const float c = (float)cnt;
            uint32_t packed = 0;
            if (rgb_on) {
                const int R = (int)__fdiv_rn(cr, c), G = (int)__fdiv_rn(cg, c), B = (int)__fdiv_rn(cb, c);
                packed = ((uint32_t)R << 16) | ((uint32_t)G << 8) | (uint32_t)B;
            }
            vox[fbase + out0 + h] = make_float4(__fdiv_rn(sx, c), __fdiv_rn(sy, c), __fdiv_rn(sz, c), __uint_as_float(packed));
        }
        h = hn; e0 = ne0; kk = nkk; rec = nrec; have = nhave;
    }
}

__global__ void __launch_bounds__(BLOCK) k_voxel_centroid_lanes(const uint32_t* __restrict__ keys,
                                                                const uint32_t* __restrict__ vals,
                                                                const float4* __restrict__ cpt, int N, int T, int Tact, int rgb_on,
                                                                FrameState* __restrict__ fs, int* __restrict__ state,
                                                                float4* __restrict__ vox, int* __restrict__ ticket, int pts_pitch) {
    CD_FRONT_PRIO();
    __shared__ int s_cnt[WAVES_PER_BLOCK];
    __shared__ int s_head[TILE];
    __shared__ int s_out0, s_ticket;
    const int F = gridDim.x / Tact;
    const int f = blockIdx.x % F, tile = take_ticket(ticket + f * TICKET_PITCH, Tact, &s_ticket), w = threadIdx.x >> 6, lane = threadIdx.x & 63;
    const int n = fs[f].n_runs;
    if (tile * TILE >= n) return;
    const size_t fbase = (size_t)f * N;
    const uint32_t* k = keys + fbase;
    const uint32_t* v = vals + fbase;
    const float4* pts = cpt + (size_t)f * pts_pitch;
    const TileHeads th = tile_voxel_heads(k, n, tile, state + (size_t)f * T, fs[f], s_cnt, s_head, s_out0);
    const int nheads = th.nheads, out0 = th.out0;
    for (int h0 = w * WAVE; h0 < nheads; h0 += BLOCK) {
        const int h = h0 + lane;
        bool alive = h < nheads;
        int e = 0, i = 0, cnt = 0;
        uint32_t key = 0, wk0 = 0, wk1 = 0, wk2 = 0, wk3 = 0, wv0 = 0, wv1 = 0, wv2 = 0, wv3 = 0;
        if (alive) {
            e = s_head[h];
            key = k[e];
            wk0 = key; wv0 = v[e];
            wk1 = wk2 = wk3 = ~key;
            if (e + 1 < n) { wk1 = k[e + 1]; wv1 = v[e + 1]; }
            if (e + 2 < n) { wk2 = k[e + 2]; wv2 = v[e + 2]; }
            if (e + 3 < n) { wk3 = k[e + 3]; wv3 = v[e + 3]; }
        }
        uint32_t nk0 = 0, nk1 = 0, nk2 = 0, nk3 = 0, nv0 = 0, nv1 = 0, nv2 = 0, nv3 = 0;
        float sx = 0.f, sy = 0.f, sz = 0.f;
        uint32_t ir = 0, ig = 0, ib = 0;
        while (ballot64(alive)) {
            const bool m0 = alive && wk0 == key, m1 = m0 && wk1 == key, m2 = m1 && wk2 == key, m3 = m2 && wk3 == key;
            const int l0 = m0 ? (int)(wv0 >> RUN_SHIFT) : 0, l1 = m1 ? (int)(wv1 >> RUN_SHIFT) : 0, l2 = m2 ? (int)(wv2 >> RUN_SHIFT) : 0, l3 = m3 ? (int)(wv3 >> RUN_SHIFT) : 0;
            const int c1 = l0, c2 = c1 + l1, c3 = c2 + l2, tot = c3 + l3;
            const int s0 = (int)(wv0 & RUN_START_MASK), s1 = (int)(wv1 & RUN_START_MASK) - c1, s2 = (int)(wv2 & RUN_START_MASK) - c2, s3 = (int)(wv3 & RUN_START_MASK) - c3;
            if (m3 && i == 0) {
                nk0 = nk1 = nk2 = nk3 = ~key;
                if (e + 4 < n) { nk0 = k[e + 4]; nv0 = v[e + 4]; }
                if (e + 5 < n) { nk1 = k[e + 5]; nv1 = v[e + 5]; }
                if (e + 6 < n) { nk2 = k[e + 6]; nv2 = v[e + 6]; }
                if (e + 7 < n) { nk3 = k[e + 7]; nv3 = v[e + 7]; }
            }
            const float4 z = make_float4(0.f, 0.f, 0.f, 0.f);
            float4 P[8];
#pragma unroll
            for (int t = 0; t < 8; ++t) {
                const int idx = i + t;
                const int off = idx >= c3 ? s3 : (idx >= c2 ? s2 : (idx >= c1 ? s1 : s0));
                P[t] = z;
                if (idx < tot && CD_IN_RANGE(off + idx >= 0 && off + idx < pts_pitch, 4u)) P[t] = pts[off + idx];
            }
#pragma unroll
            for (int t = 0; t < 8; ++t) {
                sx = __fadd_rn(sx, P[t].x); sy = __fadd_rn(sy, P[t].y); sz = __fadd_rn(sz, P[t].z);
                if (rgb_on) rgb_add(__float_as_uint(P[t].w), ir, ig, ib);
            }
            i += 8;
            if (alive && i >= tot) {
                cnt += tot;
                alive = m3 && nk0 == key;
                e += 4; i = 0;
                wk0 = nk0; wk1 = nk1; wk2 = nk2; wk3 = nk3; wv0 = nv0; wv1 = nv1; wv2 = nv2; wv3 = nv3;
            }
        }
        if (h < nheads) {
            float cr = (float)ir, cg = (float)ig, cb = (float)ib;
            if (rgb_on && cnt > 65536) rgb_replay(k, v, pts, s_head[h], n, key, cr, cg, cb);
            store_centroid(&vox[fbase + out0 + h], sx, sy, sz, cr, cg, cb, cnt, rgb_on);
        }
    }
}

void launch_crop_count(hipStream_t s, const void* in, size_t stride, int N, int F, int rgb_off, CropLimits lim, int T,
                       FrameState* fs, int* tile_cnt) {
    const int Tin = (N + TILE - 1) / TILE;
    hipLaunchKernelGGL(k_crop_count, dim3(Tin, F), dim3(BLOCK), 0, s, (const char*)in, stride, N, rgb_off, lim, T, fs, tile_cnt);
}
void launch_scan_tiles(hipStream_t s, int* counts, int rows, int T, int* totals, int total_pitch) {
    const ScanJob j{counts, totals, nullptr};
    hipLaunchKernelGGL(k_scan_tiles, dim3(rows, 1), dim3(BLOCK), 0, s, j, j, T, total_pitch);
}
void launch_scan_tiles2(hipStream_t s, const ScanJob& a, const ScanJob& b, int rows, int T, int total_pitch) {
    hipLaunchKernelGGL(k_scan_tiles, dim3(rows, 2), dim3(BLOCK), 0, s, a, b, T, total_pitch);
}
void launch_voxel_setup(hipStream_t s, FrameState* fs, int F, float leaf, const uint32_t* ghist, FrameState* mirror) {
    hipLaunchKernelGGL(k_voxel_setup, dim3(F), dim3(WAVE), 0, s, fs, leaf, ghist, mirror);
}
void launch_crop_compact(hipStream_t s, const void* in, size_t stride, int N, int pitch, int F, int rgb_off, CropLimits lim,
                         int T, float leaf, const FrameState* fs, const int* tile_off, float4* cpt, uint32_t* keys) {
    const int Tin = (N + TILE - 1) / TILE;
    hipLaunchKernelGGL(k_crop_compact, dim3(Tin, F), dim3(BLOCK), 0, s, (const char*)in, stride, N, pitch, rgb_off, lim, T, leaf,
                       fs, tile_off, cpt, keys);
}
void launch_crop_fused(hipStream_t s, const void* in, size_t stride, int N, int pitch, int F, int rgb_off, CropLimits lim,
                       int T, float leaf, KeyPack kp, FrameState* fs, int* state, float4* cpt, uint32_t* keys, int* ticket) {
    const int Tin = (N + TILE - 1) / TILE;
    hipLaunchKernelGGL(k_crop_fused, dim3(Tin * F), dim3(BLOCK), 0, s, (const char*)in, stride, N, pitch, rgb_off, lim, T, Tin,
                       leaf, kp, fs, state, cpt, keys, ticket);
}
void launch_crop_runs(hipStream_t s, const void* in, size_t stride, int N, int pitch, int F, int rgb_off, CropLimits lim,
                      int T, float leaf, KeyPack kp, FrameState* fs, unsigned long long* state, float4* cpt, uint32_t* rkeys,
                      uint32_t* rvals, uint32_t* ghist, int* ticket, int direct) {
    const int Tin = (N + TILE - 1) / TILE;
    if (direct)
        hipLaunchKernelGGL(k_crop_runs<true>, dim3(Tin * F), dim3(BLOCK), 0, s, (const char*)in, stride, N, pitch, rgb_off, lim, T, Tin,
                           leaf, kp, fs, state, cpt, rkeys, rvals, ghist, ticket);
    else
        hipLaunchKernelGGL(k_crop_runs<false>, dim3(Tin * F), dim3(BLOCK), 0, s, (const char*)in, stride, N, pitch, rgb_off, lim, T, Tin,
                           leaf, kp, fs, state, cpt, rkeys, rvals, ghist, ticket);
}
void launch_voxel_centroid(hipStream_t s, const uint32_t* keys, const uint32_t* vals, const float4* cpt, int N, int F,
                           int T, int Tact, int rgb_on, FrameState* fs, int* state, float4* vox, int* ticket) {
    hipLaunchKernelGGL(k_voxel_centroid, dim3(Tact * F), dim3(BLOCK), 0, s, keys, vals, cpt, N, T, Tact, rgb_on, fs, state, vox, ticket);
}
void launch_voxel_centroid_runs(hipStream_t s, const uint32_t* keys, const uint32_t* vals, const float4* cpt, int N, int F,
                                int T, int Tact, int rgb_on, FrameState* fs, int* state, float4* vox, int* ticket, int lanes, int pts_pitch) {
    if (lanes) {
        hipLaunchKernelGGL(k_voxel_centroid_lanes, dim3(Tact * F), dim3(BLOCK), 0, s, keys, vals, cpt, N, T, Tact, rgb_on, fs, state, vox, ticket, pts_pitch);
        return;
    }
    hipLaunchKernelGGL(k_voxel_centroid_runs, dim3(Tact * F), dim3(BLOCK), 0, s, keys, vals, cpt, N, T, Tact, rgb_on, fs, state, vox, ticket, pts_pitch);
}

}
```

Before: 208,200.

## Use wave-parallel decoupled look-back and defer scan waits past independent work

After: 207,800. No clear change (-0.2%).

```diff
diff --git a/perception_amd/csrc/common.hpp b/perception_amd/csrc/common.hpp
--- a/perception_amd/csrc/common.hpp
+++ b/perception_amd/csrc/common.hpp
@@ -3,6 +3,7 @@
 #include <stdint.h>
 
 #include "../../include/cuboid_hip.h"
+#include "scan_lookback.hpp"
 
 namespace cd {
 
@@ -309,49 +310,92 @@
     __syncthreads();
     return *s_ticket;
 }
+#ifndef CD_SCAN_WAVE
+#define CD_SCAN_WAVE 1
+#endif
+#ifndef CD_SCAN_DEFER
+#define CD_SCAN_DEFER 7
+#endif
+#define CD_SCAN_DEFER_CROP ((CD_SCAN_DEFER) & 1)
+#define CD_SCAN_DEFER_SCATTER ((CD_SCAN_DEFER) & 2)
+#define CD_SCAN_DEFER_HEADS ((CD_SCAN_DEFER) & 4)
+#ifndef CD_SCAN_WINDOW
+#define CD_SCAN_WINDOW 64
+#endif
+static_assert(CD_SCAN_WINDOW == 16 || CD_SCAN_WINDOW == 32 || CD_SCAN_WINDOW == 64, "look-back window: 16, 32 or 64 lanes");
+constexpr int SCAN_SPIN_LIMIT = 1 << 20;
+
+template <class W>
+__device__ __forceinline__ void scan_publish(W* st, size_t stride, int tile, W tot) {
+    __hip_atomic_store(st + (size_t)tile * stride, (tile == 0 ? ScanWord<W>::FLAG_PREFIX : ScanWord<W>::FLAG_TOTAL) | tot, __ATOMIC_RELAXED,
+                       __HIP_MEMORY_SCOPE_AGENT);
+}
+template <class W>
+__device__ __forceinline__ void scan_publish_prefix(W* st, size_t stride, int tile, W inclusive) {
+    if (tile > 0)
+        __hip_atomic_store(st + (size_t)tile * stride, ScanWord<W>::FLAG_PREFIX | inclusive, __ATOMIC_RELAXED, __HIP_MEMORY_SCOPE_AGENT);
+}
+template <class W>
+__device__ __forceinline__ W scan_wait_serial(W* st, size_t stride, int tile, int* gave_up) {
+    W excl = 0;
+    for (int q = tile - 1; q >= 0; --q) {
+        W v;
+        int spins = 0;
+        do {
+            v = __hip_atomic_load(st + (size_t)q * stride, __ATOMIC_RELAXED, __HIP_MEMORY_SCOPE_AGENT);
+            if (++spins > SCAN_SPIN_LIMIT) { *gave_up = 1; v = ScanWord<W>::FLAG_PREFIX; }
+        } while ((v & (ScanWord<W>::FLAG_TOTAL | ScanWord<W>::FLAG_PREFIX)) == 0);
+        excl += v & ScanWord<W>::PAYLOAD;
+        if (v & ScanWord<W>::FLAG_PREFIX) break;
+    }
+    return excl;
+}
+__device__ __forceinline__ uint32_t scan_wave_sum(uint32_t v) { return (uint32_t)wave_sum_i32((int)v); }
+__device__ __forceinline__ uint64_t scan_wave_sum(uint64_t v) { return wave_sum_u64(v); }
+template <class W>
+__device__ __forceinline__ W scan_wait_wave(W* st, int tile, int* gave_up) {
+    const int lane = threadIdx.x & 63;
+    W excl = 0;
+    for (int q0 = tile - 1; q0 >= 0; q0 -= CD_SCAN_WINDOW) {
+        const int q = q0 - lane;
+        const bool here = lane < CD_SCAN_WINDOW && q >= 0;
+        const uint64_t present = ballot64(here);
+        uint64_t again = present;
+        W v = 0;
+        int spins = 0;
+        LookbackStep step;
+        for (;;) {
+            if ((again >> lane) & 1ull) v = __hip_atomic_load(st + q, __ATOMIC_RELAXED, __HIP_MEMORY_SCOPE_AGENT);
+            step = lookback_decide(present, ballot64(here && (v & ScanWord<W>::FLAG_TOTAL) != 0), ballot64(here && (v & ScanWord<W>::FLAG_PREFIX) != 0));
+            if (step.kind != LOOKBACK_POLL) break;
+            again = step.lanes;
+            if (++spins > SCAN_SPIN_LIMIT) {
+                if (lane == 0) *gave_up = 1;
+                return excl;
+            }
+        }
+        const W mine = ((step.lanes >> lane) & 1ull) ? (W)(v & ScanWord<W>::PAYLOAD) : (W)0;
+        excl += step.lanes == 1ull ? (W)__shfl(mine, 0, 64) : scan_wave_sum(mine);
+        if (step.kind == LOOKBACK_DONE) break;
+    }
+    return excl;
+}
+template <class W>
+__device__ __forceinline__ W scan_wait(W* st, int tile, int* gave_up) {
+#if CD_SCAN_WAVE
+    return scan_wait_wave(st, tile, gave_up);
+#else
+    W excl = 0;
+    if ((threadIdx.x & 63) == 0) excl = scan_wait_serial(st, 1, tile, gave_up);
+    return (W)__shfl(excl, 0, 64);
+#endif
+}
 __device__ __forceinline__ int chained_scan(int* state, int stride, int tile, int tot, int* gave_up) {
-    unsigned* st = reinterpret_cast<unsigned*>(state);
-    const unsigned FLAG_TOTAL = 1u << 30, FLAG_PREFIX = 2u << 30, VALUE = (1u << 30) - 1u;
-    int excl = 0;
-    if (tile > 0) {
-        __hip_atomic_store(st + (size_t)tile * stride, FLAG_TOTAL | (unsigned)tot, __ATOMIC_RELAXED, __HIP_MEMORY_SCOPE_AGENT);
-        for (int q = tile - 1; q >= 0; --q) {
-            unsigned v;
-            int spins = 0;
-            do {
-                v = __hip_atomic_load(st + (size_t)q * stride, __ATOMIC_RELAXED, __HIP_MEMORY_SCOPE_AGENT);
-                if (++spins > (1 << 20)) { *gave_up = 1; v = FLAG_PREFIX; }
-            } while ((v & (FLAG_TOTAL | FLAG_PREFIX)) == 0u);
-            excl += (int)(v & VALUE);
-            if (v & FLAG_PREFIX) break;
-        }
-    }
-    __hip_atomic_store(st + (size_t)tile * stride, FLAG_PREFIX | (unsigned)(excl + tot), __ATOMIC_RELAXED, __HIP_MEMORY_SCOPE_AGENT);
-    return excl;
-}
-__device__ __forceinline__ void chained_scan2(unsigned long long* state, int tile, int tot_a, int tot_b, int* excl_a, int* excl_b,
-                                              int* gave_up) {
-    const unsigned long long FLAG_TOTAL = 1ull << 62, FLAG_PREFIX = 2ull << 62, MASK = (1ull << 31) - 1ull;
-    unsigned long long ea = 0ull, eb = 0ull;
-    if (tile > 0) {
-        __hip_atomic_store(state + tile, FLAG_TOTAL | ((unsigned long long)(unsigned)tot_b << 31) | (unsigned long long)(unsigned)tot_a,
-                           __ATOMIC_RELAXED, __HIP_MEMORY_SCOPE_AGENT);
-        for (int q = tile - 1; q >= 0; --q) {
-            unsigned long long v;
-            int spins = 0;
-            do {
-                v = __hip_atomic_load(state + q, __ATOMIC_RELAXED, __HIP_MEMORY_SCOPE_AGENT);
-                if (++spins > (1 << 20)) { *gave_up = 1; v = FLAG_PREFIX; }
-            } while ((v & (FLAG_TOTAL | FLAG_PREFIX)) == 0ull);
-            ea += v & MASK;
-            eb += (v >> 31) & MASK;
-            if (v & FLAG_PREFIX) break;
-        }
-    }
-    __hip_atomic_store(state + tile, FLAG_PREFIX | ((eb + (unsigned long long)(unsigned)tot_b) << 31) | (ea + (unsigned long long)(unsigned)tot_a),
-                       __ATOMIC_RELAXED, __HIP_MEMORY_SCOPE_AGENT);
-    *excl_a = (int)ea;
-    *excl_b = (int)eb;
+    uint32_t* st = reinterpret_cast<uint32_t*>(state);
+    scan_publish(st, (size_t)stride, tile, (uint32_t)tot);
+    const uint32_t excl = scan_wait_serial(st, (size_t)stride, tile, gave_up);
+    scan_publish_prefix(st, (size_t)stride, tile, excl + (uint32_t)tot);
+    return (int)excl;
 }
 __device__ __forceinline__ float plane_dist(float a, float b, float c, float d, float x, float y, float z) {
     return fabsf(__fadd_rn(__fadd_rn(__fmul_rn(a, x), __fmul_rn(b, y)), __fadd_rn(__fmul_rn(c, z), d)));
diff --git a/perception_amd/csrc/k_plane.hip b/perception_amd/csrc/k_plane.hip
--- a/perception_amd/csrc/k_plane.hip
+++ b/perception_amd/csrc/k_plane.hip
@@ -335,16 +335,20 @@
     }
     if (lane == 0) s_cnt[w] = wtot;
     __syncthreads();
-    if (threadIdx.x == 0) {
-        int tot = 0;
-        for (int k = 0; k < WAVES_PER_BLOCK; ++k) tot += s_cnt[k];
-        const int excl = chained_scan(state, 1, tile, tot, &fs[0].scan_stalled);
-        s_excl = excl;
-        if ((tile + 1) * TILE >= n) fs[0].n_plane = excl + tot;
+    int tot = 0, wpos = 0;
+    for (int k = 0; k < WAVES_PER_BLOCK; ++k) { if (k < w) wpos += s_cnt[k]; tot += s_cnt[k]; }
+    uint32_t* const st = reinterpret_cast<uint32_t*>(state);
+    if (threadIdx.x == 0) scan_publish(st, 1, tile, (uint32_t)tot);
+    if (w == 0) {
+        const int excl = (int)scan_wait(st, tile, &fs[0].scan_stalled);
+        if (lane == 0) {
+            scan_publish_prefix(st, 1, tile, (uint32_t)(excl + tot));
+            s_excl = excl;
+            if ((tile + 1) * TILE >= n) fs[0].n_plane = excl + tot;
+        }
     }
     __syncthreads();
-    int pos = s_excl;
-    for (int k = 0; k < w; ++k) pos += s_cnt[k];
+    int pos = s_excl + wpos;
     const uint64_t lt = lanemask_lt();
 #pragma unroll
     for (int j = 0; j < ITEMS; ++j) {
diff --git a/perception_amd/csrc/k_sort.hip b/perception_amd/csrc/k_sort.hip
--- a/perception_amd/csrc/k_sort.hip
+++ b/perception_amd/csrc/k_sort.hip
@@ -34,8 +34,12 @@
     return 0;
 }
 #define SORT_PHASE(k) { __syncthreads(); if (threadIdx.x == 0) { const unsigned long long t_ = wall_clock64(); atomicAdd(&g_sort_dbg[k], t_ - t0_); t0_ = t_; } }
+#define SORT_WAIT_BEGIN() const unsigned long long tw_ = wall_clock64();
+#define SORT_WAIT_END() if (threadIdx.x == 0) atomicAdd(&g_sort_dbg[4], wall_clock64() - tw_);
 #else
 #define SORT_PHASE(k)
+#define SORT_WAIT_BEGIN()
+#define SORT_WAIT_END()
 #endif
 constexpr int SORT_MAX_PASSES = 4;
 constexpr int GHIST_TILES = 4;
@@ -106,6 +110,7 @@
     const uint64_t lt = lanemask_lt();
     const KeyGrid g = key_grid(fs[f]);
     uint32_t key[ITEMS], rank[ITEMS], val[ITEMS];
+    uint32_t bin_run = 0;
 #pragma unroll
     for (int j = 0; j < ITEMS; ++j) {
         const int e = base + j * WAVE;
@@ -152,8 +157,14 @@
         }
         if (lane == 63) { s_ws[w] = inc; s_gs[w] = ginc; }
         s_bstart[d] = inc - run;
+#if CD_SCAN_DEFER_SCATTER
+        scan_publish(reinterpret_cast<uint32_t*>(state) + (size_t)f * T * RADIX + d, RADIX, tile, run);
+        bin_run = run;
+        s_goff[d] = ginc - tot;
+#else
         const int before = chained_scan(state + (size_t)f * T * RADIX + d, RADIX, tile, (int)run, &fs[f].scan_stalled);
         s_goff[d] = ginc - tot + (uint32_t)before;
+#endif
     }
     __syncthreads();
     if (threadIdx.x < RADIX) {
@@ -176,6 +187,16 @@
             }
         }
     }
+#if CD_SCAN_DEFER_SCATTER
+    if (threadIdx.x < RADIX) {
+        uint32_t* const st = reinterpret_cast<uint32_t*>(state) + (size_t)f * T * RADIX + threadIdx.x;
+        SORT_WAIT_BEGIN()
+        const uint32_t before = scan_wait_serial(st, RADIX, tile, &fs[f].scan_stalled);
+        SORT_WAIT_END()
+        scan_publish_prefix(st, RADIX, tile, before + bin_run);
+        s_goff[threadIdx.x] += before;
+    }
+#endif
     __syncthreads();
     SORT_PHASE(2)
     const int cnt = min(SCATTER_TILE, n - tile * SCATTER_TILE);
@@ -247,24 +268,40 @@
     __syncthreads();
     int pos = 0, nheads = 0;
     for (int q = 0; q < SORT_WAVES; ++q) { if (q < w) pos += s_cnt[q]; nheads += s_cnt[q]; }
-    if (threadIdx.x == 0) {
-        const int excl = chained_scan(state + (size_t)f * T, 1, tile, nheads, &fs[f].scan_stalled);
-        s_out0 = excl;
-        if ((tile + 1) * SORT_TILE >= n) fs[f].n_runs = excl + nheads;
-    }
-    __syncthreads();
-    const int out0 = s_out0;
+    uint32_t* const st = reinterpret_cast<uint32_t*>(state) + (size_t)f * T;
+    if (threadIdx.x == 0) scan_publish(st, 1, tile, (uint32_t)nheads);
+    auto wait_prefix = [&]() {
+        if (w == 0) {
+            const int excl = (int)scan_wait(st, tile, &fs[f].scan_stalled);
+            if (lane == 0) {
+                scan_publish_prefix(st, 1, tile, (uint32_t)(excl + nheads));
+                s_out0 = excl;
+                if ((tile + 1) * SORT_TILE >= n) fs[f].n_runs = excl + nheads;
+            }
+        }
+        __syncthreads();
+    };
     const uint64_t lt = lanemask_lt();
+    auto store_runs = [&](int rpos) {
+#pragma unroll
+        for (int j = 0; j < ITEMS; ++j) {
+            if ((heads[j] >> lane) & 1ull) {
+                const uint64_t above = lane == 63 ? 0ull : heads[j] & ~((2ull << lane) - 1ull);
+                const int next = above ? __ffsll((long long)above) - 1 : nvalid[j];
+                const size_t o = fbase + (size_t)(rpos + __popcll(heads[j] & lt));
+                kout[o] = key[j];
+                vout[o] = (uint32_t)(base + j * WAVE) | ((uint32_t)(next - lane) << RUN_SHIFT);
+            }
+            rpos += __popcll(heads[j]);
+        }
+    };
+#if !CD_SCAN_DEFER_HEADS
+    wait_prefix();
+    store_runs(s_out0 + pos);
+#endif
 #pragma unroll
     for (int j = 0; j < ITEMS; ++j) {
         const bool is_head = (heads[j] >> lane) & 1ull;
-        if (is_head) {
-            const uint64_t above = lane == 63 ? 0ull : heads[j] & ~((2ull << lane) - 1ull);
-            const int next = above ? __ffsll((long long)above) - 1 : nvalid[j];
-            const size_t o = fbase + (size_t)(out0 + pos + __popcll(heads[j] & lt));
-            kout[o] = key[j];
-            vout[o] = (uint32_t)(base + j * WAVE) | ((uint32_t)(next - lane) << RUN_SHIFT);
-        }
         if (heads[j]) {
             const int first = __ffsll((long long)heads[j]) - 1;
             for (int p = 0; p < npass; ++p) {
@@ -279,13 +316,16 @@
                 if (is_head) atomicAdd(&s_h[p][d], 1u);
             }
         }
-        pos += __popcll(heads[j]);
     }
     __syncthreads();
     for (int q = threadIdx.x; q < npass * RADIX; q += SORT_BLOCK) {
         const uint32_t c = (&s_h[0][0])[q];
         if (c) atomicAdd(&ghist[(size_t)f * SORT_MAX_PASSES * RADIX + q], c);
     }
+#if CD_SCAN_DEFER_HEADS
+    wait_prefix();
+    store_runs(s_out0 + pos);
+#endif
 }
 
 int launch_radix_sort_runs(hipStream_t s, uint32_t* const key[2], uint32_t* const val[2], int N, int F, int T, int Tact, int Tscat, int npass,
diff --git a/perception_amd/csrc/k_voxel.hip b/perception_amd/csrc/k_voxel.hip
--- a/perception_amd/csrc/k_voxel.hip
+++ b/perception_amd/csrc/k_voxel.hip
@@ -1,6 +1,24 @@
 #include "kernels.hpp"
 
 namespace cd {
+
+#ifdef CD_SORTDBG
+__device__ unsigned long long g_scan_dbg[8];
+extern "C" int cd_debug_scan(unsigned long long* out, int reset) {
+    if (hipMemcpyFromSymbol(out, HIP_SYMBOL(g_scan_dbg), sizeof(g_scan_dbg)) != hipSuccess) return -1;
+    if (reset) { static unsigned long long z[8]; (void)hipMemcpyToSymbol(HIP_SYMBOL(g_scan_dbg), z, sizeof(z)); }
+    return 0;
+}
+#define SCAN_DBG_LIFE_BEGIN() const unsigned long long dbg_t0_ = wall_clock64();
+#define SCAN_DBG_WAIT_BEGIN() const unsigned long long dbg_w0_ = wall_clock64();
+#define SCAN_DBG_WAIT_END(k) if (threadIdx.x == 0) atomicAdd(&g_scan_dbg[k], wall_clock64() - dbg_w0_);
+#define SCAN_DBG_LIFE_END(k) if (threadIdx.x == 0) { atomicAdd(&g_scan_dbg[(k) + 1], wall_clock64() - dbg_t0_); atomicAdd(&g_scan_dbg[(k) + 2], 1ull); }
+#else
+#define SCAN_DBG_LIFE_BEGIN()
+#define SCAN_DBG_WAIT_BEGIN()
+#define SCAN_DBG_WAIT_END(k)
+#define SCAN_DBG_LIFE_END(k)
+#endif
 
 template <int R>
 __device__ __forceinline__ void load_rows(const char* __restrict__ in, size_t stride, size_t fbase, int first, int N, int rgb_off,
@@ -267,17 +285,23 @@
     box.reduce_wave(s_mn[w], s_mx[w], lane);
     if (lane == 0) s_cnt[w] = wtot;
     __syncthreads();
+    int tot = 0, wpos = 0;
+    for (int k = 0; k < WAVES_PER_BLOCK; ++k) { if (k < w) wpos += s_cnt[k]; tot += s_cnt[k]; }
+    uint32_t* const st = reinterpret_cast<uint32_t*>(state) + (size_t)f * T;
     if (threadIdx.x == 0) {
-        int tot = 0;
-        for (int k = 0; k < WAVES_PER_BLOCK; ++k) tot += s_cnt[k];
-        const int excl = chained_scan(state + (size_t)f * T, 1, tile, tot, &fs[f].crop_overflow);
-        s_excl = excl;
-        if (tile == Tin - 1) fs[f].n_c = excl + tot;
+        scan_publish(st, 1, tile, (uint32_t)tot);
         CropBox::commit(fs[f], s_mn, s_mx, tot);
     }
-    __syncthreads();
-    int pos = s_excl;
-    for (int k = 0; k < w; ++k) pos += s_cnt[k];
+    if (w == 0) {
+        const int excl = (int)scan_wait(st, tile, &fs[f].crop_overflow);
+        if (lane == 0) {
+            scan_publish_prefix(st, 1, tile, (uint32_t)(excl + tot));
+            s_excl = excl;
+            if (tile == Tin - 1) fs[f].n_c = excl + tot;
+        }
+    }
+    __syncthreads();
+    int pos = s_excl + wpos;
     const float inv = __fdiv_rn(1.0f, leaf);
     const uint64_t lt = lanemask_lt();
     bool over = false;
@@ -306,6 +330,7 @@
                                                      float4* __restrict__ cpt, uint32_t* __restrict__ rkeys, uint32_t* __restrict__ rvals,
                                                      uint32_t* __restrict__ ghist, int* __restrict__ ticket) {
     CD_FRONT_PRIO();
+    SCAN_DBG_LIFE_BEGIN()
     __shared__ int s_cnt[WAVES_PER_BLOCK], s_rcnt[WAVES_PER_BLOCK];
     __shared__ float s_mn[WAVES_PER_BLOCK][3], s_mx[WAVES_PER_BLOCK][3];
     __shared__ uint32_t s_h[4][RADIX];
@@ -352,40 +377,58 @@
     box.reduce_wave(s_mn[w], s_mx[w], lane);
     if (lane == 0) { s_cnt[w] = wtot; s_rcnt[w] = rtot; }
     __syncthreads();
-    if (threadIdx.x == 0) {
-        int tot = 0, rt = 0;
-        for (int k = 0; k < WAVES_PER_BLOCK; ++k) { tot += s_cnt[k]; rt += s_rcnt[k]; }
-        int excl = 0, rexcl = 0;
-        chained_scan2(state + (size_t)f * T, tile, tot, rt, &excl, &rexcl, &fs[f].crop_overflow);
-        s_excl = excl; s_rexcl = rexcl;
-        if (tile == Tin - 1) { fs[f].n_c = excl + tot; fs[f].n_runs = rexcl + rt; }
-        CropBox::commit(fs[f], s_mn, s_mx, tot);
-    }
-    __syncthreads();
-    const int rexcl0 = s_rexcl;
-    int pos = s_excl, rpos = rexcl0;
-    for (int k = 0; k < w; ++k) { pos += s_cnt[k]; rpos += s_rcnt[k]; }
+    int tot = 0, rt = 0, wpos = 0, wrpos = 0;
+    for (int k = 0; k < WAVES_PER_BLOCK; ++k) {
+        if (k < w) { wpos += s_cnt[k]; wrpos += s_rcnt[k]; }
+        tot += s_cnt[k]; rt += s_rcnt[k];
+    }
+    uint64_t* const st = reinterpret_cast<uint64_t*>(state) + (size_t)f * T;
+    if (threadIdx.x == 0) scan_publish(st, 1, tile, scan_pack2(tot, rt));
+    auto wait_prefix = [&]() {
+        if (w == 0) {
+            SCAN_DBG_WAIT_BEGIN()
+            const uint64_t excl = scan_wait(st, tile, &fs[f].crop_overflow);
+            SCAN_DBG_WAIT_END(0)
+            if (lane == 0) {
+                scan_publish_prefix(st, 1, tile, excl + scan_pack2(tot, rt));
+                s_excl = scan_first(excl); s_rexcl = scan_second(excl);
+                if (tile == Tin - 1) { fs[f].n_c = scan_first(excl) + tot; fs[f].n_runs = scan_second(excl) + rt; }
+            }
+        }
+    };
     const uint64_t lt = lanemask_lt();
-#pragma unroll
-    for (int j = 0; j < ITEMS; ++j) {
-        const bool kept = (bal[j] >> lane) & 1ull;
-        const int r = pos + __popcll(bal[j] & lt);
-        if (!DIRECT && kept && r < pitch) cpt[obase + r] = make_float4(px[j], py[j], pz[j], __uint_as_float(pc[j]));
-        const bool is_head = (heads[j] >> lane) & 1ull;
-        if (is_head) {
-            const uint64_t stop = (~bal[j] | heads[j]) & (lane == 63 ? 0ull : ~((2ull << lane) - 1ull));
-            const int next = stop ? __ffsll((long long)stop) - 1 : 64;
-            const int ro = rpos + __popcll(heads[j] & lt);
-            const uint32_t key = s_key[w * WAVE_SPAN + j * WAVE + lane];
-            s_rk[ro - rexcl0] = (unsigned short)(w * WAVE_SPAN + j * WAVE + lane);
-            if (ro < pitch && CD_IN_RANGE(ro >= 0, 5u)) {
-                rkeys[obase + ro] = key;
-                rvals[obase + ro] = (uint32_t)(DIRECT ? base + j * WAVE + lane : r) | ((uint32_t)(next - lane) << RUN_SHIFT);
-            }
-        }
-        pos += __popcll(bal[j]);
-        rpos += __popcll(heads[j]);
-    }
+    auto emit = [&](bool number, bool store, int pos, int rpos) {
+        int lpos = wrpos;
+#pragma unroll
+        for (int j = 0; j < ITEMS; ++j) {
+            const bool kept = (bal[j] >> lane) & 1ull;
+            const int r = pos + __popcll(bal[j] & lt);
+            if (store && !DIRECT && kept && r < pitch) cpt[obase + r] = make_float4(px[j], py[j], pz[j], __uint_as_float(pc[j]));
+            const bool is_head = (heads[j] >> lane) & 1ull;
+            if (is_head) {
+                const int rl = lpos + __popcll(heads[j] & lt);
+                if (number) s_rk[rl] = (unsigned short)(w * WAVE_SPAN + j * WAVE + lane);
+                const int ro = rpos + __popcll(heads[j] & lt);
+                if (store && ro < pitch && CD_IN_RANGE(ro >= 0, 5u)) {
+                    const uint64_t stop = (~bal[j] | heads[j]) & (lane == 63 ? 0ull : ~((2ull << lane) - 1ull));
+                    const int next = stop ? __ffsll((long long)stop) - 1 : 64;
+                    rkeys[obase + ro] = s_key[w * WAVE_SPAN + j * WAVE + lane];
+                    rvals[obase + ro] = (uint32_t)(DIRECT ? base + j * WAVE + lane : r) | ((uint32_t)(next - lane) << RUN_SHIFT);
+                }
+            }
+            pos += __popcll(bal[j]);
+            rpos += __popcll(heads[j]);
+            lpos += __popcll(heads[j]);
+        }
+    };
+#if CD_SCAN_DEFER_CROP
+    emit(true, false, 0, 0);
+#else
+    wait_prefix();
+    if (threadIdx.x == 0) CropBox::commit(fs[f], s_mn, s_mx, tot);
+    __syncthreads();
+    emit(true, true, s_excl + wpos, s_rexcl + wrpos);
+#endif
     if (__ballot(over) != 0ull && lane == 0) fs[f].crop_overflow = 1;
     __syncthreads();
     {
@@ -412,6 +455,13 @@
         const uint32_t c = (&s_h[0][0])[q];
         if (c) atomicAdd(&ghist[(size_t)f * 4 * RADIX + q], c);
     }
+#if CD_SCAN_DEFER_CROP
+    if (threadIdx.x == 0) CropBox::commit(fs[f], s_mn, s_mx, tot);
+    wait_prefix();
+    __syncthreads();
+    emit(false, true, s_excl + wpos, s_rexcl + wrpos);
+#endif
+    SCAN_DBG_LIFE_END(0)
 }
 
 template <int R>
@@ -441,6 +491,15 @@
 }
 
 struct TileHeads { int nheads, out0; };
+__device__ __forceinline__ int tile_voxel_out0(int n, int tile, int nheads, int* state, FrameState& s) {
+    uint32_t* const st = reinterpret_cast<uint32_t*>(state);
+    const int excl = (int)scan_wait(st, tile, &s.scan_stalled);
+    if (threadIdx.x == 0) {
+        scan_publish_prefix(st, 1, tile, (uint32_t)(excl + nheads));
+        if ((tile + 1) * TILE >= n) s.n_v = excl + nheads;
+    }
+    return excl;
+}
 __device__ __forceinline__ TileHeads tile_voxel_heads(const uint32_t* k, int n, int tile, int* state, FrameState& s,
                                                       int (&s_cnt)[WAVES_PER_BLOCK], int (&s_head)[TILE], int& s_out0) {
     const int w = threadIdx.x >> 6, lane = threadIdx.x & 63;
@@ -454,11 +513,15 @@
     __syncthreads();
     int pos = 0, nheads = 0;
     for (int q = 0; q < WAVES_PER_BLOCK; ++q) { if (q < w) pos += s_cnt[q]; nheads += s_cnt[q]; }
-    if (threadIdx.x == 0) {
-        const int excl = chained_scan(state, 1, tile, nheads, &s.scan_stalled);
-        s_out0 = excl;
-        if ((tile + 1) * TILE >= n) s.n_v = excl + nheads;
-    }
+    if (threadIdx.x == 0) scan_publish(reinterpret_cast<uint32_t*>(state), 1, tile, (uint32_t)nheads);
+#if !CD_SCAN_DEFER_HEADS
+    if (w == 0) {
+        SCAN_DBG_WAIT_BEGIN()
+        const int excl = tile_voxel_out0(n, tile, nheads, state, s);
+        SCAN_DBG_WAIT_END(3)
+        if (lane == 0) s_out0 = excl;
+    }
+#endif
     const uint64_t lt = lanemask_lt();
 #pragma unroll
     for (int j = 0; j < ITEMS; ++j) {
@@ -466,7 +529,11 @@
         pos += __popcll(bal[j]);
     }
     __syncthreads();
+#if CD_SCAN_DEFER_HEADS
+    return {nheads, -1};
+#else
     return {nheads, s_out0};
+#endif
 }
 
 __device__ __forceinline__ void rgb_add(uint32_t u, uint32_t& ir, uint32_t& ig, uint32_t& ib) {
@@ -514,13 +581,17 @@
     const uint32_t* k = keys + fbase;
     const uint32_t* v = vals + fbase;
     const TileHeads th = tile_voxel_heads(k, n, tile, state + (size_t)f * T, fs[f], s_cnt, s_head, s_out0);
-    const int nheads = th.nheads, out0 = th.out0;
-    const int quad = threadIdx.x >> 2, ql = threadIdx.x & 3;
-    for (int h = quad; h < nheads; h += BLOCK / 4) {
+    const int nheads = th.nheads;
+    int out0 = th.out0;
+    const int w = threadIdx.x >> 6, ql = threadIdx.x & 3;
+    for (int hb = w * (WAVE / 4); hb < nheads; hb += BLOCK / 4) {
+        const int h = hb + ((threadIdx.x & 63) >> 2);
+        const bool on = h < nheads;
+        float sx = 0.f, sy = 0.f, sz = 0.f, cr = 0.f, cg = 0.f, cb = 0.f;
+        int cnt = 0;
+        if (on) {
         const int e0 = s_head[h];
         const uint32_t key = k[e0];
-        float sx = 0.f, sy = 0.f, sz = 0.f, cr = 0.f, cg = 0.f, cb = 0.f;
-        int cnt = 0;
         for (int e = e0;; e += 4) {
             const int me = e + ql;
             uint32_t kk = ~key, vv = 0;
@@ -543,8 +614,11 @@
 #undef CD_ACC
             if (!m3) break;
         }
-        if (ql == 0) store_centroid(&vox[fbase + out0 + h], sx, sy, sz, cr, cg, cb, cnt, rgb_on);
-    }
+        }
+        if (out0 < 0) out0 = tile_voxel_out0(n, tile, nheads, state + (size_t)f * T, fs[f]);
+        if (on && ql == 0) store_centroid(&vox[fbase + out0 + h], sx, sy, sz, cr, cg, cb, cnt, rgb_on);
+    }
+    if (w == 0 && out0 < 0) tile_voxel_out0(n, tile, nheads, state + (size_t)f * T, fs[f]);
 }
 
 __global__ void __launch_bounds__(BLOCK) k_voxel_centroid_runs(const uint32_t* __restrict__ keys,
@@ -565,7 +639,8 @@
     const uint32_t* v = vals + fbase;
     const float4* pts = cpt + (size_t)f * pts_pitch;
     const TileHeads th = tile_voxel_heads(k, n, tile, state + (size_t)f * T, fs[f], s_cnt, s_head, s_out0);
-    const int nheads = th.nheads, out0 = th.out0;
+    const int nheads = th.nheads;
+    int out0 = th.out0;
     const int quad = threadIdx.x >> 2, ql = threadIdx.x & 3;
     int h = quad, e0 = 0;
     uint32_t kk = 0, rec = 0;
@@ -575,7 +650,8 @@
         have = e0 + ql < n;
         if (have) { kk = k[e0 + ql]; rec = v[e0 + ql]; }
     }
-    while (h < nheads) {
+    while (ballot64(h < nheads)) {
+        const bool on = h < nheads;
         const int hn = h + BLOCK / 4;
         int ne0 = 0;
         uint32_t nkk = 0, nrec = 0;
@@ -589,6 +665,8 @@
         float sx = 0.f, sy = 0.f, sz = 0.f;
         uint32_t ir = 0, ig = 0, ib = 0;
         int cnt = 0;
+        float cr = 0.f, cg = 0.f, cb = 0.f;
+        if (on) {
 #define CD_ADD(P, J)                                                                                   \
         {                                                                                              \
             sx = __fadd_rn(sx, quad_bcast<J>(P.x)); sy = __fadd_rn(sy, quad_bcast<J>(P.y));            \
@@ -639,9 +717,11 @@
         }
 #undef CD_RUN
 #undef CD_ADD
-        float cr = (float)ir, cg = (float)ig, cb = (float)ib;
+        cr = (float)ir; cg = (float)ig; cb = (float)ib;
         if (rgb_on && cnt > 65536) rgb_replay(k, v, pts, e0, n, key, cr, cg, cb);
-        if (ql == 0) {
+        }
+        if (out0 < 0) out0 = tile_voxel_out0(n, tile, nheads, state + (size_t)f * T, fs[f]);
+        if (on && ql == 0) {
             const float c = (float)cnt;
             uint32_t packed = 0;
             if (rgb_on) {
@@ -652,6 +732,7 @@
         }
         h = hn; e0 = ne0; kk = nkk; rec = nrec; have = nhave;
     }
+    if (threadIdx.x < WAVE && out0 < 0) tile_voxel_out0(n, tile, nheads, state + (size_t)f * T, fs[f]);
 }
 
 __global__ void __launch_bounds__(BLOCK) k_voxel_centroid_lanes(const uint32_t* __restrict__ keys,
@@ -660,6 +741,7 @@
                                                                 FrameState* __restrict__ fs, int* __restrict__ state,
                                                                 float4* __restrict__ vox, int* __restrict__ ticket, int pts_pitch) {
     CD_FRONT_PRIO();
+    SCAN_DBG_LIFE_BEGIN()
     __shared__ int s_cnt[WAVES_PER_BLOCK];
     __shared__ int s_head[TILE];
     __shared__ int s_out0, s_ticket;
@@ -672,7 +754,8 @@
     const uint32_t* v = vals + fbase;
     const float4* pts = cpt + (size_t)f * pts_pitch;
     const TileHeads th = tile_voxel_heads(k, n, tile, state + (size_t)f * T, fs[f], s_cnt, s_head, s_out0);
-    const int nheads = th.nheads, out0 = th.out0;
+    const int nheads = th.nheads;
+    int out0 = th.out0;
     for (int h0 = w * WAVE; h0 < nheads; h0 += BLOCK) {
         const int h = h0 + lane;
         bool alive = h < nheads;
@@ -724,12 +807,19 @@
                 wk0 = nk0; wk1 = nk1; wk2 = nk2; wk3 = nk3; wv0 = nv0; wv1 = nv1; wv2 = nv2; wv3 = nv3;
             }
         }
+        if (out0 < 0) {
+            SCAN_DBG_WAIT_BEGIN()
+            out0 = tile_voxel_out0(n, tile, nheads, state + (size_t)f * T, fs[f]);
+            SCAN_DBG_WAIT_END(3)
+        }
         if (h < nheads) {
             float cr = (float)ir, cg = (float)ig, cb = (float)ib;
             if (rgb_on && cnt > 65536) rgb_replay(k, v, pts, s_head[h], n, key, cr, cg, cb);
             store_centroid(&vox[fbase + out0 + h], sx, sy, sz, cr, cg, cb, cnt, rgb_on);
         }
     }
+    if (w == 0 && out0 < 0) tile_voxel_out0(n, tile, nheads, state + (size_t)f * T, fs[f]);
+    SCAN_DBG_LIFE_END(3)
 }
 
 void launch_crop_count(hipStream_t s, const void* in, size_t stride, int N, int F, int rgb_off, CropLimits lim, int T,
diff --git a/perception_amd/csrc/scan_lookback.hpp b/perception_amd/csrc/scan_lookback.hpp
--- /dev/null
+++ b/perception_amd/csrc/scan_lookback.hpp
@@ -0,0 +1,56 @@
+#pragma once
+#include <stdint.h>
+
+#if defined(__HIPCC__) || defined(__CUDACC__)
+#define CD_SCAN_HD __host__ __device__ __forceinline__
+#else
+#define CD_SCAN_HD inline
+#endif
+
+namespace cd {
+
+template <class W> struct ScanWord;
+template <> struct ScanWord<uint32_t> {
+    static constexpr uint32_t FLAG_TOTAL = 1u << 30, FLAG_PREFIX = 2u << 30, PAYLOAD = (1u << 30) - 1u;
+};
+template <> struct ScanWord<uint64_t> {
+    static constexpr uint64_t FLAG_TOTAL = 1ull << 62, FLAG_PREFIX = 2ull << 62, PAYLOAD = (1ull << 62) - 1ull;
+};
+CD_SCAN_HD uint64_t scan_pack2(int a, int b) { return ((uint64_t)(uint32_t)b << 31) | (uint64_t)(uint32_t)a; }
+CD_SCAN_HD int scan_first(uint64_t payload) { return (int)(payload & ((1ull << 31) - 1ull)); }
+CD_SCAN_HD int scan_second(uint64_t payload) { return (int)((payload >> 31) & ((1ull << 31) - 1ull)); }
+
+enum LookbackKind : int {
+    LOOKBACK_DONE = 0,
+    LOOKBACK_FURTHER = 1,
+    LOOKBACK_POLL = 2
+};
+struct LookbackStep {
+    LookbackKind kind;
+    uint64_t lanes;
+};
+CD_SCAN_HD LookbackStep lookback_decide(uint64_t present, uint64_t total, uint64_t prefix) {
+    const uint64_t published = total | prefix;
+    if (prefix) {
+        const uint64_t nearest = prefix & (~prefix + 1ull);
+        const uint64_t nearer = nearest - 1ull;
+        const uint64_t waiting = nearer & ~published;
+        if (waiting) return {LOOKBACK_POLL, waiting};
+        return {LOOKBACK_DONE, nearer | nearest};
+    }
+    const uint64_t waiting = present & ~published;
+    if (waiting) return {LOOKBACK_POLL, waiting};
+    return {LOOKBACK_FURTHER, present};
+}
+
+template <class W>
+CD_SCAN_HD W lookback_serial(const W* words, int tile) {
+    W excl = 0;
+    for (int q = tile - 1; q >= 0; --q) {
+        excl += words[q] & ScanWord<W>::PAYLOAD;
+        if (words[q] & ScanWord<W>::FLAG_PREFIX) break;
+    }
+    return excl;
+}
+
+}
diff --git a/perception_amd/csrc/scan_lookback_check.cpp b/perception_amd/csrc/scan_lookback_check.cpp
--- /dev/null
+++ b/perception_amd/csrc/scan_lookback_check.cpp
@@ -0,0 +1,227 @@
+#include <cstdio>
+#include <cstdlib>
+#include <vector>
+
+#include "scan_lookback.hpp"
+
+using namespace cd;
+
+struct Rng {
+    uint64_t s;
+    uint64_t next() {
+        uint64_t z = (s += 0x9E3779B97F4A7C15ull);
+        z = (z ^ (z >> 30)) * 0xBF58476D1CE4E5B9ull;
+        z = (z ^ (z >> 27)) * 0x94D049BB133111EBull;
+        return z ^ (z >> 31);
+    }
+    int below(int n) { return (int)(next() % (uint64_t)n); }
+};
+
+static long long g_bad = 0;
+#define CHECK(c, ...)                                                   \
+    do {                                                                \
+        if (!(c)) {                                                     \
+            if (g_bad++ < 20) { std::printf("FAIL %s: ", #c); std::printf(__VA_ARGS__); std::printf("\n"); } \
+        }                                                               \
+    } while (0)
+
+enum { U = 0, TOT = 1, PRE = 2 };
+static void check_window(const int* lane_state, int n) {
+    uint64_t present = 0, total = 0, prefix = 0;
+    for (int l = 0; l < n; ++l) {
+        present |= 1ull << l;
+        if (lane_state[l] == TOT) total |= 1ull << l;
+        if (lane_state[l] == PRE) prefix |= 1ull << l;
+    }
+    LookbackKind kind = LOOKBACK_FURTHER;
+    uint64_t lanes = 0, waiting = 0;
+    int l = 0;
+    for (; l < n; ++l) {
+        if (lane_state[l] == U) waiting |= 1ull << l;
+        lanes |= 1ull << l;
+        if (lane_state[l] == PRE) break;
+    }
+    if (waiting) { kind = LOOKBACK_POLL; lanes = waiting; }
+    else if (l < n) kind = LOOKBACK_DONE;
+    const LookbackStep s = lookback_decide(present, total, prefix);
+    CHECK(s.kind == kind && s.lanes == lanes, "n %d got %d %llx want %d %llx", n, (int)s.kind, (unsigned long long)s.lanes, (int)kind,
+          (unsigned long long)lanes);
+}
+static long long windows(Rng& r) {
+    long long cnt = 0;
+    int st[64];
+    for (int n = 1; n <= 64; ++n) {
+        for (int l = 0; l < n; ++l) st[l] = TOT;
+        check_window(st, n); ++cnt;
+        for (int l = 0; l < n; ++l) st[l] = U;
+        check_window(st, n); ++cnt;
+        for (int p = 0; p < n; ++p) {
+            for (int behind = 0; behind < 3; ++behind) {
+                for (int l = 0; l < n; ++l) st[l] = l < p ? TOT : (l == p ? PRE : behind);
+                check_window(st, n); ++cnt;
+            }
+            for (int u = 0; u < n; ++u) {
+                if (u == p) continue;
+                for (int l = 0; l < n; ++l) st[l] = l == p ? PRE : (l == u ? U : TOT);
+                check_window(st, n); ++cnt;
+            }
+        }
+    }
+    for (int it = 0; it < 400000; ++it) {
+        const int n = 1 + r.below(64), bias = r.below(4);
+        for (int l = 0; l < n; ++l) {
+            const int x = r.below(8);
+            st[l] = bias == 0 ? x % 3 : (bias == 1 ? (x == 0 ? PRE : TOT) : (bias == 2 ? (x == 0 ? U : (x == 1 ? PRE : TOT)) : (x < 4 ? U : TOT)));
+        }
+        check_window(st, n); ++cnt;
+    }
+    return cnt;
+}
+
+template <class W>
+struct WaveWait {
+    int tile = 0, width = 64, q0 = 0;
+    bool done = false, fresh = true;
+    uint64_t present = 0, again = 0;
+    W v[64];
+    W excl = 0;
+    long long polls = 0;
+    void start(int t, int w) {
+        tile = t; width = w; q0 = t - 1; done = q0 < 0; fresh = true; excl = 0; polls = 0;
+    }
+    void round(const W* words) {
+        if (done) return;
+        if (fresh) {
+            present = 0;
+            for (int l = 0; l < 64; ++l) {
+                v[l] = 0;
+                if (l < width && q0 - l >= 0) present |= 1ull << l;
+            }
+            again = present;
+            fresh = false;
+        }
+        uint64_t total = 0, prefix = 0;
+        for (int l = 0; l < 64; ++l) {
+            if ((again >> l) & 1ull) v[l] = words[q0 - l];
+            const bool here = (present >> l) & 1ull;
+            if (here && (v[l] & ScanWord<W>::FLAG_TOTAL)) total |= 1ull << l;
+            if (here && (v[l] & ScanWord<W>::FLAG_PREFIX)) prefix |= 1ull << l;
+        }
+        ++polls;
+        const LookbackStep s = lookback_decide(present, total, prefix);
+        if (s.kind == LOOKBACK_POLL) {
+            CHECK((s.lanes & ~present) == 0 && s.lanes != 0, "poll outside the window");
+            for (int l = 0; l < 64; ++l)
+                if ((s.lanes >> l) & 1ull) CHECK(v[l] == 0, "a published lane is read again");
+            again = s.lanes;
+            return;
+        }
+        for (int l = 0; l < 64; ++l)
+            if ((s.lanes >> l) & 1ull) excl += v[l] & ScanWord<W>::PAYLOAD;
+        if (s.kind == LOOKBACK_DONE) { done = true; return; }
+        q0 -= width;
+        fresh = true;
+        CHECK(q0 >= 0, "the look-back walked past tile 0");
+        if (q0 < 0) done = true;
+    }
+};
+
+template <class W> static W make_payload(Rng& r);
+template <> uint32_t make_payload<uint32_t>(Rng& r) { return r.below(7) == 0 ? 0u : (uint32_t)r.below(2049); }
+template <> uint64_t make_payload<uint64_t>(Rng& r) { return r.below(7) == 0 ? 0ull : scan_pack2(r.below(2049), r.below(2049)); }
+
+template <class W>
+static long long rows(Rng& r) {
+    long long cnt = 0;
+    const int tiles[] = {0, 1, 63, 64, 65, 129};
+    for (int it = 0; it < 3000; ++it) {
+        const int tile = it < 600 ? tiles[it % 6] : r.below(400);
+        std::vector<W> words(tile + 1), tot(tile + 1);
+        const int solid = tile ? r.below(tile) : 0, sprinkle = r.below(3);
+        W run = 0;
+        for (int q = 0; q < tile; ++q) {
+            tot[q] = make_payload<W>(r);
+            run += tot[q];
+            const bool pre = q <= solid || (sprinkle && r.below(sprinkle * 20) == 0);
+            words[q] = pre ? (ScanWord<W>::FLAG_PREFIX | run) : (ScanWord<W>::FLAG_TOTAL | tot[q]);
+        }
+        const W want = lookback_serial(words.data(), tile);
+        CHECK(want == run, "serial definition, tile %d", tile);
+        for (int width = 16; width <= 64; width *= 2) {
+            WaveWait<W> w;
+            w.start(tile, width);
+            for (int guard = 0; !w.done && guard < 1000; ++guard) w.round(words.data());
+            CHECK(w.done && w.excl == want, "tile %d width %d: got %llu want %llu", tile, width, (unsigned long long)w.excl, (unsigned long long)want);
+            ++cnt;
+        }
+    }
+    return cnt;
+}
+
+template <class W>
+static void store_word(std::vector<W>& words, int q, W nw) {
+    const W old = words[q];
+    const int of = (int)(old >> (sizeof(W) * 8 - 2)), nf = (int)(nw >> (sizeof(W) * 8 - 2));
+    CHECK(nf > of && (nf == 1 || nf == 2), "word %d moves from flag %d to %d", q, of, nf);
+    words[q] = nw;
+}
+template <class W>
+static long long schedule(Rng& r, int T, int width, long long* polls) {
+    std::vector<W> words(T, 0), tot(T), want(T);
+    std::vector<int> phase(T, 0);
+    std::vector<WaveWait<W>> wave(T);
+    W run = 0;
+    for (int q = 0; q < T; ++q) { tot[q] = make_payload<W>(r); want[q] = run; run += tot[q]; }
+    const int bias = r.below(3);
+    int started = 0, finished = 0;
+    long long steps = 0;
+    while (finished < T) {
+        CHECK(++steps < 100000000ll, "schedule does not end");
+        if (steps >= 100000000ll) break;
+        int q;
+        if (started < T && (started == finished || r.below(bias == 0 ? 2 : 4) == 0)) { phase[started++] = 3; continue; }
+        else {
+            q = bias == 2 && r.below(4) ? started - 1 - r.below(started < 8 ? started : 8) : r.below(started);
+            int tries = 0;
+            while (phase[q] == 2 && tries++ < 4) q = r.below(started);
+            if (phase[q] == 2) {
+                if (bias == 1 && r.below(2)) { q = started - 1; while (q >= 0 && phase[q] == 2) --q; }
+                else { q = 0; while (q < started && phase[q] == 2) ++q; }
+                if (q < 0 || q >= started) continue;
+            }
+        }
+        if (phase[q] == 3) {
+            store_word<W>(words, q, (q == 0 ? ScanWord<W>::FLAG_PREFIX : ScanWord<W>::FLAG_TOTAL) | tot[q]);
+            wave[q].start(q, width);
+            phase[q] = 1;
+            continue;
+        }
+        wave[q].round(words.data());
+        if (wave[q].done) {
+            CHECK(wave[q].excl == want[q], "T %d tile %d: got %llu want %llu", T, q, (unsigned long long)wave[q].excl, (unsigned long long)want[q]);
+            if (q > 0) store_word<W>(words, q, ScanWord<W>::FLAG_PREFIX | (wave[q].excl + tot[q]));
+            *polls += wave[q].polls;
+            phase[q] = 2;
+            ++finished;
+        }
+    }
+    return 1;
+}
+
+int main(int argc, char** argv) {
+    const int per = argc > 1 ? std::atoi(argv[1]) : 300;
+    Rng r{20240611ull};
+    const long long nw = windows(r);
+    const long long nr = rows<uint32_t>(r) + rows<uint64_t>(r);
+    long long ns = 0, polls = 0;
+    const int Ts[] = {1, 2, 64, 65, 66, 150};
+    for (int T : Ts)
+        for (int it = 0; it < per; ++it) {
+            const int width = 16 << (it % 3);
+            ns += schedule<uint32_t>(r, T, width, &polls);
+            ns += schedule<uint64_t>(r, T, width, &polls);
+        }
+    if (g_bad) { std::printf("%lld differences\n", g_bad); return 1; }
+    std::printf("ok %lld %lld %lld %lld\n", nw, nr, ns, polls);
+    return 0;
+}
```
